# genlm/genlm-backend

Measured on AMD Instinct MI355X. Metric: particles/sec + logprob-kernel HBM GB/s (% of 8 TB/s), 1024 particles gpt2, higher is better.
Workload: dtype f32

## Files before the change

### genlm-backend_amd/_lib.py

```python
import ctypes as C
import os

_HERE = os.path.dirname(os.path.abspath(__file__))
LIB_PATH = os.path.join(_HERE, "libglb_hip.so")

ABI_VERSION = 9
GLB_OK, GLB_EINVAL, GLB_EUNSUPPORTED, GLB_EHIP, GLB_ENOSPC = 0, 1, 2, 3, 4
F32, BF16, F16 = 0, 1, 2
MASK_NONE, MASK_BITS, MASK_F32, MASK_PREPARED = 0, 1, 2, 3
RNG_NONE, RNG_PHILOX, RNG_NOISE = 0, 1, 2
STEP_HW_EXP = 1
GEMM_BIAS, GEMM_BIAS_GELU_TANH = 0, 1
GEMM_FORM_LARGE, GEMM_FORM_SMALL = 1, 2


class GlbError(RuntimeError):
    def __init__(self, code, msg):
        super().__init__(f"glb error {code}: {msg}")
        self.code = code


class StepArgs(C.Structure):
    _fields_ = [
        ("struct_size", C.c_uint32),
# ... 91 lines not shown
        ("workspace_bytes", C.c_size_t),
    ]


class KvPlanArgs(C.Structure):
    _fields_ = [
        ("struct_size", C.c_uint32),
        ("n", C.c_int64), ("n_rows", C.c_int64), ("cap", C.c_int64),
        ("group_of", C.c_void_p), ("rep", C.c_void_p), ("n_groups", C.c_void_p),
        ("old_row", C.c_void_p),
        ("old_row_by_context", C.c_int32),
        ("lengths", C.c_void_p),
        ("row_stamps", C.c_void_p),
        ("call_no", C.c_int64),
        ("row_tok", C.c_void_p), ("row_len", C.c_void_p),
        ("row_hash", C.c_void_p),
        ("group_hash", C.c_void_p),
        ("tokens", C.c_void_p),
        ("starts", C.c_void_p),
        ("out_group_row", C.c_void_p), ("out_logits_row", C.c_void_p), ("out_rows_a", C.c_void_p), ("out_ctx_a", C.c_void_p),
        ("out_pos_a", C.c_void_p), ("out_ctx_b", C.c_void_p), ("out_rows_b", C.c_void_p), ("out_copy_src", C.c_void_p),
        ("out_copy_len", C.c_void_p), ("out_ctx_of_row", C.c_void_p), ("out_pos_of_row", C.c_void_p),
        ("out_row_of_context", C.c_void_p), ("out_head", C.c_void_p),
        ("workspace", C.c_void_p),
        ("workspace_bytes", C.c_size_t),
    ]


class KvPlanChunkArgs(C.Structure):
    _fields_ = [
        ("struct_size", C.c_uint32),
        ("plan", KvPlanArgs),
        ("old_keep", C.c_void_p),
        ("out_n_new_a", C.c_void_p), ("out_n_new_of_row", C.c_void_p),
    ]


KV_CHUNK_MAX = 16


class MT19937(C.Structure):
    _fields_ = [("mt", C.c_uint32 * 624), ("idx", C.c_int32)]


MT_POLY_WORDS = 312


class MtRowsArgs(C.Structure):
    _fields_ = [
        ("struct_size", C.c_uint32),
        ("window", C.c_void_p), ("window_out", C.c_void_p), ("polys", C.c_void_p),
        ("n_small", C.c_int32), ("n_big", C.c_int32),
        ("vocab", C.c_int64), ("max_draw_rows", C.c_int64),
        ("n_draw", C.c_void_p),
        ("n_out_rows", C.c_int64),
        ("row_slot", C.c_void_p),
        ("out", C.c_void_p), ("out_ld", C.c_int64),
        ("workspace", C.c_void_p), ("workspace_bytes", C.c_size_t),
        ("reuse_windows", C.c_int32), ("rows_from", C.c_void_p), ("rows_from_ld", C.c_int64),
    ]


class GemmArgs(C.Structure):
    _fields_ = [
        ("struct_size", C.c_uint32),
        ("m", C.c_int64), ("n", C.c_int64), ("k", C.c_int64),
        ("a", C.c_void_p), ("lda", C.c_int64),
        ("w_split", C.c_void_p),
        ("bias", C.c_void_p),
        ("c", C.c_void_p), ("ldc", C.c_int64),
        ("epilogue", C.c_int32),
    ]


class PackedPlanArgs(C.Structure):
    _fields_ = [
        ("struct_size", C.c_uint32),
        ("n_tokens", C.c_int64), ("n_contexts", C.c_int64), ("n_sel", C.c_int64), ("n_groups", C.c_int64),
        ("n_pre", C.c_int64), ("n_tail_rows", C.c_int64), ("pos_cap", C.c_int64),
        ("tokens", C.c_void_p), ("starts", C.c_void_p), ("lengths", C.c_void_p), ("sel", C.c_void_p), ("grp", C.c_void_p),
        ("group_starts", C.c_void_p), ("group_lens", C.c_void_p), ("group_segments", C.c_void_p),
        ("group_ids", C.c_void_p), ("group_pos", C.c_void_p),
        ("segments", C.c_void_p), ("ids", C.c_void_p), ("pos", C.c_void_p), ("last", C.c_void_p), ("ends", C.c_void_p),
    ]


class LoraJob(C.Structure):
    _fields_ = [
        ("struct_size", C.c_uint32),
        ("w_dtype", C.c_int32), ("ab_dtype", C.c_int32), ("w_transposed", C.c_int32),
        ("n_out", C.c_int64), ("k_in", C.c_int64), ("r", C.c_int64),
        ("w", C.c_void_p), ("ldw", C.c_int64),
        ("a", C.c_void_p), ("lda", C.c_int64),
        ("b", C.c_void_p), ("ldb", C.c_int64),
        ("scale", C.c_float),
        ("out", C.c_void_p), ("ldo", C.c_int64),
    ]


class LoraRowsEntry(C.Structure):
    _fields_ = [
        ("struct_size", C.c_uint32),
        ("ab_dtype", C.c_int32),
        ("n_out", C.c_int64), ("k_in", C.c_int64), ("r", C.c_int64),
        ("a", C.c_void_p), ("lda", C.c_int64),
        ("b", C.c_void_p), ("ldb", C.c_int64),
        ("scale", C.c_float),
    ]


class LoraRowsArgs(C.Structure):
    _fields_ = [
        ("struct_size", C.c_uint32),
        ("dtype", C.c_int32),
        ("m", C.c_int64), ("n", C.c_int64), ("k", C.c_int64),
        ("x", C.c_void_p), ("ldx", C.c_int64),
        ("y", C.c_void_p), ("ldy", C.c_int64),
        ("row_slot", C.c_void_p),
        ("table", C.c_void_p),
        ("n_slots", C.c_int32), ("n_modules", C.c_int32), ("module", C.c_int32), ("r_max", C.c_int32),
        ("workspace", C.c_void_p), ("workspace_bytes", C.c_size_t),
    ]


class W4Args(C.Structure):
    _fields_ = [
        ("struct_size", C.c_uint32),
        ("dtype", C.c_int32), ("transposed", C.c_int32),
        ("n", C.c_int64), ("k", C.c_int64),
        ("w", C.c_void_p), ("ldw", C.c_int64),
        ("codebook", C.POINTER(C.c_float)),
        ("image", C.c_void_p), ("image_bytes", C.c_size_t),
    ]


class W4GemmArgs(C.Structure):
    _fields_ = [
        ("struct_size", C.c_uint32),
        ("dtype", C.c_int32),
        ("m", C.c_int64), ("n", C.c_int64), ("k", C.c_int64),
        ("x", C.c_void_p), ("ldx", C.c_int64),
        ("image", C.c_void_p),
        ("codebook", C.POINTER(C.c_float)),
        ("bias", C.c_void_p),
        ("y", C.c_void_p), ("ldy", C.c_int64),
        ("workspace", C.c_void_p), ("workspace_bytes", C.c_size_t),
    ]


DFA_COUNTERS = 4


class DfaArgs(C.Structure):
    _fields_ = [
        ("struct_size", C.c_uint32),
        ("n_states", C.c_int32), ("start", C.c_int32), ("eos_id", C.c_int32),
        ("delta", C.c_void_p), ("accepting", C.c_void_p), ("live", C.c_void_p),
        ("vocab", C.c_int64),
        ("tok_bytes", C.c_void_p), ("n_bytes", C.c_int64), ("tok_ptr", C.c_void_p), ("skip", C.c_void_p),
        ("n", C.c_int64),
        ("tokens", C.c_void_p), ("ld", C.c_int64), ("from_", C.c_void_p), ("to", C.c_void_p),
        ("state_in", C.c_void_p), ("state_out", C.c_void_p),
        ("bank", C.c_void_p), ("bank_ld", C.c_int64), ("capacity", C.c_int64),
        ("row_of_state", C.c_void_p), ("work", C.c_void_p), ("counters", C.c_void_p),
        ("max_work", C.c_int64),
        ("done", C.c_void_p), ("out_rows", C.c_void_p),
# ... 214 lines not shown
        ("seq_start", C.c_void_p), ("n_seq", C.c_int64),
        ("out_seq_logp", C.c_void_p), ("out_seq_logZ", C.c_void_p), ("out_seq_logp_masked", C.c_void_p),
    ]


class TopkArgs(C.Structure):
    _fields_ = [
        ("struct_size", C.c_uint32),
        ("logits", C.c_void_p), ("dtype", C.c_int32),
        ("n_rows", C.c_int64), ("vocab", C.c_int64), ("ld", C.c_int64),
        ("logit_scale", C.c_float), ("k", C.c_int32),
        ("mask_kind", C.c_int32), ("mask", C.c_void_p), ("mask_ld", C.c_int64), ("n_masks", C.c_int64),
        ("row_mask_id", C.c_void_p),
        ("out_token", C.c_void_p), ("out_logp", C.c_void_p), ("out_logp_masked", C.c_void_p),
        ("out_lse", C.c_void_p), ("out_logZ", C.c_void_p),
    ]


class ByteLmArgs(C.Structure):
    _fields_ = [
        ("struct_size", C.c_uint32), ("width", C.c_int32),
        ("n_groups", C.c_int64), ("n_nodes", C.c_int64), ("root", C.c_int32),
        ("child_ptr", C.c_void_p), ("child_idx", C.c_void_p), ("child_sym", C.c_void_p), ("leaf_token", C.c_void_p),
        ("node", C.c_void_p), ("alive", C.c_void_p), ("u", C.c_void_p), ("w", C.c_void_p),
        ("sel", C.c_void_p), ("mass", C.c_void_p), ("fresh", C.c_void_p),
        ("out_parent", C.c_void_p), ("out_token", C.c_void_p), ("out_node", C.c_void_p), ("out_alive", C.c_void_p),
        ("out_u", C.c_void_p), ("out_w", C.c_void_p), ("out_spawned", C.c_void_p), ("out_n_spawned", C.c_void_p),
        ("byte", C.c_void_p), ("out_next", C.c_void_p), ("out_logZ", C.c_void_p), ("logp", C.c_void_p),
    ]


class TruncateArgs(C.Structure):
    _fields_ = [
        ("struct_size", C.c_uint32),
        ("logits", C.c_void_p), ("dtype", C.c_int32),
        ("n_rows", C.c_int64), ("vocab", C.c_int64), ("ld", C.c_int64),
        ("logit_scale", C.c_float),
        ("mask_kind", C.c_int32), ("mask", C.c_void_p), ("mask_ld", C.c_int64), ("n_masks", C.c_int64),
        ("row_mask_id", C.c_void_p),
        ("top_k", C.c_int64), ("top_p", C.c_float), ("log_min_p", C.c_float),
        ("out_bits", C.c_void_p), ("out_ld", C.c_int64),
        ("out_threshold", C.c_void_p), ("out_kept", C.c_void_p), ("out_logmass", C.c_void_p),
    ]


_vp, _i32, _i64, _f32, _sz = C.c_void_p, C.c_int32, C.c_int64, C.c_float, C.c_size_t
SYMBOLS = {
    "glb_version": (C.c_char_p, []),
    "glb_abi_version": (C.c_int, []),
    "glb_last_error": (C.c_int, [C.c_char_p, _sz]),
    "glb_device_count": (C.c_int, []),
    "glb_step_workspace_bytes": (_sz, [_i64, _i64, _i64, _i64]),
    "glb_logprob_mask_sample": (C.c_int, [C.POINTER(StepArgs), _vp]),
    "glb_logprob_mask_sample_timed": (C.c_int, [C.POINTER(StepArgs), _vp, _vp, _vp]),
    "glb_workspace_init": (C.c_int, [_vp, _sz, _vp]),
    "glb_workspace_release": (C.c_int, [_vp]),
    "glb_workspace_check": (C.c_int, [_vp, _vp]),
    "glb_workspace_error_word": (_vp, [_vp]),
    "glb_set_spin_limit": (C.c_int, [C.c_uint64]),
    "glb_mask_prepared_bytes": (_sz, [_i64, _i64]),
    "glb_mask_prepare": (C.c_int, [_vp, _i64, _i64, _i64, _i32, _vp, _sz, _vp]),
    "glb_mask_prepare_rows": (C.c_int, [_vp, _i64, _i64, _i64, _i32, _vp, _i64, _vp, _sz, _vp]),
    "glb_log_softmax_workspace_bytes": (_sz, [_i64, _i64]),
    "glb_log_softmax_rows": (C.c_int, [_vp, _i32, _i64, _i64, _i64, _f32, _vp, _i32, _i64, _vp, _vp, _sz, _vp]),
    "glb_mask_f32_to_bits": (C.c_int, [_vp, _i64, _i64, _i64, _vp, _i64, _vp, _vp]),
    "glb_group_contexts_workspace": (_sz, [_i64]),
    "glb_group_contexts": (C.c_int, [_vp, _vp, _vp, _i64, _vp, _vp, _vp, _vp, _vp, _sz, _vp]),
    "glb_hash_contexts": (C.c_int, [_vp, _vp, _vp, _i64, _vp, _vp]),
    "glb_match_prefixes": (C.c_int, [_vp, _vp, _vp, _i64, _vp, _vp, _vp, _i64, _vp, _vp, _vp]),
    "glb_gather_padded": (C.c_int, [_vp, _vp, _vp, _vp, _i64, _vp, _i64, _i64, _i64, _vp, _vp, _vp, _vp, _vp]),
    "glb_gather_kv_padded": (C.c_int, [_vp, _vp, _i64, _vp, _i64, _i64, _i64, _i64, _i32, _vp, _vp]),
    "glb_particles_advance": (C.c_int, [_vp, _i64, _vp, _vp, _vp, _vp, _vp, _i64, _i32, _i32, _vp, _vp]),
    "glb_normalize_weights": (C.c_int, [_vp, _i64, _vp, _vp, _vp]),
    "glb_kv_append": (C.c_int, [_vp, _vp, _vp, _vp, _i64, _i64, _i64, _i64, _i64, _i64, _i32, _vp]),
    "glb_kv_gather_rows": (C.c_int, [_vp, _vp, _i64, _i64, _i64, _i64, _i64, _i64, _vp, _vp, _i32, _vp]),
    "glb_gather_rows_i32": (C.c_int, [_vp, _i64, _vp, _i64, _i64, _vp, _i64, _vp]),
    "glb_match_rows": (C.c_int, [_vp, _vp, _vp, _vp, _vp, _i64, _vp, _vp, _vp, _i64, _i64, _vp, _vp, _vp]),
    "glb_slab_attention": (C.c_int, [_vp, _i64, _i64, _vp, _i64, _i64, _vp, _i64, _i64, _vp, _vp, _vp, _i64, _i64, _i64, _i64, _i64,
                                     _f32, _i32, _vp, _vp]),
    "glb_short_attention": (C.c_int, [_vp, C.POINTER(C.c_int64), _vp, C.POINTER(C.c_int64), _vp, C.POINTER(C.c_int64), _vp, _i64, _i64,
                                      _i64, _i64, _i64, _i64, _i64, _i64, _f32, _i32, _vp, _vp]),
    "glb_short_attention_packed": (C.c_int, [_vp, _i64, _i64, _vp, _i64, _i64, _vp, _i64, _i64, _vp, _i64, _i64, _i64, _i64, _i64,
                                             _i64, _f32, _i32, _vp, _vp, _vp]),
    "glb_kv_plan_workspace": (_sz, [_i64, _i64]),
    "glb_kv_plan": (C.c_int, [C.POINTER(KvPlanArgs), _vp]),
    "glb_match_prefix_rows": (C.c_int, [_vp, _vp, _vp, _vp, _vp, _i64, _vp, _vp, _vp, _i64, _i64, _i32, _vp, _vp, _vp, _vp]),
    "glb_kv_plan_chunk": (C.c_int, [C.POINTER(KvPlanChunkArgs), _vp]),
    "glb_slab_attention_chunk": (C.c_int, [_vp, C.POINTER(C.c_int64), _vp, C.POINTER(C.c_int64), _vp, C.POINTER(C.c_int64), _vp, _vp,
                                           _vp, _vp, _vp, _i64, _i64, _i64, _i64, _i64, _i64, _i64, _f32, _i32, _vp, _vp]),
    "glb_trie_workspace": (_sz, [_i64, _i64]),
    "glb_trie_reduce": (C.c_int, [_vp, _i64, _i64, _i64, _i64, _i64, _vp, _vp, _vp, _vp, _vp, _i32, _i32, _vp, _i64, _vp, _sz,
                                  _vp]),
    "glb_trie_workspace_ex": (_sz, [_i64, _i64]),
    "glb_trie_masses": (C.c_int, [C.POINTER(TrieArgs), _vp]),
    "glb_trie_rows_workspace": (_sz, [_i64, C.POINTER(TriePlan)]),
    "glb_trie_rows": (C.c_int, [C.POINTER(TrieRowsArgs), C.POINTER(TriePlan), _vp]),
    "glb_resample_workspace": (_sz, [_i64]),
    "glb_resample_systematic": (C.c_int, [_vp, _i64, C.c_uint64, C.c_uint64, _vp, _vp, _vp, _sz, _vp]),
    "glb_mt19937_seed": (None, [C.POINTER(MT19937), C.c_uint64]),
    "glb_mt19937_exponential_f32": (C.c_int, [C.POINTER(MT19937), _vp, _i64]),
    "glb_mt19937_window": (C.c_int, [C.c_uint64, _vp]),
    "glb_mt19937_jump_polys": (C.c_int, [_i64, _i32, _i32, _vp]),
    "glb_mt19937_jump_host": (C.c_int, [_vp, _vp, _vp]),
    "glb_mt19937_rows_workspace": (_sz, [_i64, _i32]),
    "glb_mt19937_exponential_rows": (C.c_int, [C.POINTER(MtRowsArgs), _vp]),
    "glb_comm_unique_id": (C.c_int, [_vp]),
    "glb_comm_init": (C.c_int, [_vp, _i32, _i32, C.POINTER(C.c_void_p)]),
    "glb_allgather_f32": (C.c_int, [_vp, _vp, _i64, _vp, _vp]),
    "glb_comm_destroy": (C.c_int, [_vp]),
    "glb_gemm_split_bytes": (_sz, [_i64, _i64]),
    "glb_gemm_split_weights": (C.c_int, [_vp, _i64, _i64, _i64, _vp, _sz, _vp]),
    "glb_gemm_f32_split": (C.c_int, [C.POINTER(GemmArgs), _vp]),
    "glb_gemm_split_pick": (C.c_int, [_i64, _i64, _i64, C.c_int, C.POINTER(C.c_int)]),
    "glb_gemm_f32_split_form": (C.c_int, [C.POINTER(GemmArgs), C.c_int, _vp]),
    "glb_gemm_f32_split_residual": (C.c_int, [C.POINTER(GemmArgs), _vp, _i64, C.c_int, _vp]),
    "glb_packed_plan": (C.c_int, [C.POINTER(PackedPlanArgs), _vp]),
    "glb_gemm_split_blocks_per_cu": (C.c_int, [C.c_int, C.POINTER(C.c_int)]),
    "glb_gemm_split_form_blocks_per_cu": (C.c_int, [C.c_int, C.c_int, C.POINTER(C.c_int)]),
    "glb_lora_merge_workspace_bytes": (_sz, [_i32]),
    "glb_lora_merge": (C.c_int, [C.POINTER(LoraJob), _i32, _vp, _sz, _vp]),
    "glb_lora_rows_table_bytes": (_sz, [_i32, _i32]),
    "glb_lora_rows_table_upload": (C.c_int, [C.POINTER(LoraRowsEntry), _i32, _i32, _vp, _sz, _vp]),
    "glb_lora_rows_workspace_bytes": (_sz, [_i64, _i32]),
    "glb_lora_rows": (C.c_int, [C.POINTER(LoraRowsArgs), _vp]),
    "glb_w4_bytes": (_sz, [_i64, _i64]),
    "glb_w4_quantize": (C.c_int, [C.POINTER(W4Args), _vp]),
    "glb_w4_dequantize": (C.c_int, [C.POINTER(W4Args), _vp]),
    "glb_w4_gemm_max_rows": (C.c_int, []),
    "glb_w4_gemm_workspace_bytes": (_sz, [_i64, _i64, _i64]),
    "glb_w4_gemm": (C.c_int, [C.POINTER(W4GemmArgs), _vp]),
    "glb_dfa_bank_init": (C.c_int, [C.POINTER(DfaArgs), _vp]),
    "glb_dfa_advance": (C.c_int, [C.POINTER(DfaArgs), _vp]),
    "glb_dfa_claim_rows": (C.c_int, [C.POINTER(DfaArgs), _vp]),
    "glb_dfa_fill_masks": (C.c_int, [C.POINTER(DfaArgs), _vp]),
    "glb_dfa_mask_ids": (C.c_int, [C.POINTER(DfaArgs), _vp]),
    "glb_dfa_bank_rows": (_i64, [_sz, _i64, _i64]),
    "glb_dfa_weight_bank_init": (C.c_int, [C.POINTER(DfaWeightArgs), _vp]),
    "glb_dfa_fill_weights": (C.c_int, [C.POINTER(DfaWeightArgs), _vp]),
    "glb_dfa_weight_bank_rows": (_i64, [_sz, _i64, _i64]),
    "glb_dfa_evict_bank_init": (C.c_int, [C.POINTER(DfaEvictArgs), _vp]),
    "glb_dfa_evict_serve": (C.c_int, [C.POINTER(DfaEvictArgs), _vp]),
    "glb_dfa_backward": (C.c_int, [C.POINTER(DfaPushArgs), _vp]),
    "glb_dfa_push_weights": (C.c_int, [C.POINTER(DfaPushArgs), _vp]),
    "glb_dfa_refine": (C.c_int, [C.POINTER(DfaMinArgs), _vp]),
    "glb_dfa_quotient": (C.c_int, [C.POINTER(DfaMinArgs), _vp]),
    "glb_fsa_product_round": (C.c_int, [C.POINTER(FsaProductArgs), _vp]),
    "glb_fsa_live": (C.c_int, [C.POINTER(FsaProductArgs), _vp]),
    "glb_nfa_closure": (C.c_int, [C.POINTER(NfaArgs), _vp]),
    "glb_nfa_subset_round": (C.c_int, [C.POINTER(NfaArgs), _vp]),
    "glb_lazy_init": (C.c_int, [C.POINTER(LazyArgs), _vp]),
    "glb_lazy_advance": (C.c_int, [C.POINTER(LazyArgs), _vp]),
    "glb_lazy_serve": (C.c_int, [C.POINTER(LazyArgs), _vp]),
    "glb_pda_init": (C.c_int, [C.POINTER(PdaArgs), _vp]),
    "glb_pda_advance": (C.c_int, [C.POINTER(PdaArgs), _vp]),
    "glb_pda_serve": (C.c_int, [C.POINTER(PdaArgs), _vp]),
    "glb_conj_init": (C.c_int, [C.POINTER(ConjArgs), _vp]),
    "glb_conj_unpack": (C.c_int, [C.POINTER(ConjArgs), _vp]),
    "glb_conj_number": (C.c_int, [C.POINTER(ConjArgs), _vp]),
    "glb_conj_serve": (C.c_int, [C.POINTER(ConjArgs), _vp]),
    "glb_importance_workspace_bytes": (_sz, [_i64, _i64, _i64]),
    "glb_importance_step": (C.c_int, [C.POINTER(ImportanceArgs), _vp]),
    "glb_score_rows": (C.c_int, [C.POINTER(ScoreArgs), _vp]),
    "glb_score_seq_sums": (C.c_int, [_vp, _i64, _vp, _i64, _vp, _vp]),
    "glb_topk_rows": (C.c_int, [C.POINTER(TopkArgs), _vp]),
    "glb_truncate_rows": (C.c_int, [C.POINTER(TruncateArgs), _vp]),
    "glb_beam_select": (C.c_int, [_vp, _vp, _vp, _vp, _i64, _i32, _i32, _vp, _vp, _vp, _vp]),
    "glb_bytelm_children": (C.c_int, [C.POINTER(ByteLmArgs), _vp]),
    "glb_bytelm_extend": (C.c_int, [C.POINTER(ByteLmArgs), _vp]),
    "glb_bytelm_next": (C.c_int, [C.POINTER(ByteLmArgs), _vp]),
    "glb_philox4x32_10": (None, [C.POINTER(C.c_uint32), C.POINTER(C.c_uint32), C.POINTER(C.c_uint32)]),
}

_lib = None


def load():
    global _lib
    if _lib is not None:
        return _lib
    if not os.path.exists(LIB_PATH):
        raise ImportError(
            f"{LIB_PATH} not found: build it with `make -C genlm-backend_amd/csrc -j8` "
            "(or `python -c 'import __graft_entry__ as g; g.build()'`). There is no CPU fallback."
        )
    import torch

    lib = C.CDLL(LIB_PATH)
    for name, (res, args) in SYMBOLS.items():
        fn = getattr(lib, name)
        fn.restype = res
        fn.argtypes = args
    if lib.glb_abi_version() != ABI_VERSION:
        raise ImportError(f"libglb_hip.so ABI {lib.glb_abi_version()} != {ABI_VERSION}")
    _lib = lib
    return lib


def last_error():
    buf = C.create_string_buffer(512)
# ... 8 lines not shown
```

### genlm-backend_amd/csrc/glb_kv.hip

```cpp
#include <hip/hip_runtime.h>

#include <climits>

#include "../../include/glb.h"
#include "glb_common.hpp"

namespace {

__device__ inline uint64_t ctx_hash_step(uint64_t h, uint32_t v) {
  h ^= v;
  h *= 0x100000001b3ull;
  return h ^ (h >> 29);
}

__global__ __launch_bounds__(64) void match_rows_kernel(const int32_t *tok, const int64_t *st, const int32_t *len,
                                                        const int32_t *rep, const int32_t *n_groups, const int32_t *row_tok,
                                                        const int32_t *row_len, const uint64_t *row_hash, int32_t R,
                                                        int32_t cap, int32_t *out_old, uint64_t *out_hash) {
  const int u = blockIdx.x, lane = threadIdx.x;
  if (u >= *n_groups) return;
  const int i = rep[u];
  const int32_t L = len[i];
  const int32_t *t = tok + st[i];
  uint64_t h = 0xcbf29ce484222325ull, h_par = h;
// ... 717 lines not shown
    const int qc = live ? qi : nq - 1;
    const int g = qc / a.Lq, t = qc - g * a.Lq, h = hk * G + g;
    float qf[EPV];
    unpack16<DT>(q_raw, qf);
    if (q0 + PP < nq) q_raw = *reinterpret_cast<const u32x4 *>(q_addr(qi + PP));
    const uint32_t vis = vis_t[t];
    float sc[KMAX];
    float m = -__builtin_huge_valf();
#pragma unroll
    for (int p = 0; p < KMAX; ++p) {
      sc[p] = -__builtin_huge_valf();
      if (p < a.Lk) {
        float s = 0.0f;
        if constexpr (KREG) {
#pragma unroll
          for (int k = 0; k < EPV; ++k) s = __builtin_fmaf(qf[k], kr[p][k], s);
        } else {
          const float *kp = Ks + p * DH + i * EPV;
#pragma unroll
          for (int k = 0; k < EPV; ++k) s = __builtin_fmaf(qf[k], kp[k], s);
        }
        s = slot_sum<LP>(s) * a.scale;
        sc[p] = ((vis >> p) & 1u) ? s : -__builtin_huge_valf();
        m = fmaxf(m, sc[p]);
      }
    }
    float l = 0.0f, acc[EPV];
#pragma unroll
    for (int k = 0; k < EPV; ++k) acc[k] = 0.0f;
#pragma unroll
    for (int p = 0; p < KMAX; ++p) {
      if (p < a.Lk) {
        const float w = ((vis >> p) & 1u) ? __expf(sc[p] - m) : 0.0f;
        const float *vp = Vs + p * DH + i * EPV;
        l += w;
#pragma unroll
        for (int k = 0; k < EPV; ++k) acc[k] = __builtin_fmaf(w, vp[k], acc[k]);
      }
    }
    if (live) {
      const float inv = l > 0.0f ? 1.0f / l : 0.0f;
#pragma unroll
      for (int k = 0; k < EPV; ++k) acc[k] *= inv;
      *reinterpret_cast<u32x4 *>(a.out + ((((int64_t)u * a.Lq + t) * a.H + h) * DH + i * EPV) * ES) = pack16v<DT>(acc);
    }
  }
}

template <int DT, int DH>
hipError_t launch_short_rows(const ShortArgs &a, hipStream_t s) {
  const dim3 grid((unsigned)((int64_t)a.U * a.Hkv)), block(64);
  const size_t lds = (size_t)2 * a.Lk * DH * sizeof(float) + (size_t)a.Lq * sizeof(uint32_t);
  if (a.Lk <= 16) hipLaunchKernelGGL((short_attention_rows_kernel<DT, DH, 16>), grid, block, lds, s, a);
  else hipLaunchKernelGGL((short_attention_rows_kernel<DT, DH, 32>), grid, block, lds, s, a);
  return hipGetLastError();
}

template <int DT>
hipError_t launch_short_attention(const ShortArgs &a, int head_dim, hipStream_t s) {
  if (a.Lk <= 32 && a.Lq <= 2048 && (int64_t)a.U * a.Hkv <= 0x7fffffffll) {
    if (head_dim == 64) return launch_short_rows<DT, 64>(a, s);
    if (head_dim == 128) return launch_short_rows<DT, 128>(a, s);
    if (head_dim == 32) return launch_short_rows<DT, 32>(a, s);
    if (head_dim == 16) return launch_short_rows<DT, 16>(a, s);
    return hipErrorInvalidValue;
  }
  const dim3 grid((unsigned)((int64_t)a.U * a.H * a.Lq)), block(64);
  if (head_dim == 64) hipLaunchKernelGGL((short_attention_kernel<DT, 64>), grid, block, 0, s, a);
  else if (head_dim == 128) hipLaunchKernelGGL((short_attention_kernel<DT, 128>), grid, block, 0, s, a);
  else if (head_dim == 32) hipLaunchKernelGGL((short_attention_kernel<DT, 32>), grid, block, 0, s, a);
  else if (head_dim == 16) hipLaunchKernelGGL((short_attention_kernel<DT, 16>), grid, block, 0, s, a);
  else return hipErrorInvalidValue;
  return hipGetLastError();
}

struct PackedArgs {
  const char *q, *k, *v;
  char *out;
  const int32_t *plan;
  uint32_t *err;
  int64_t q_sr, q_sh, k_sr, k_sh, v_sr, v_sh;
  int32_t S, M, H, Hkv, max_keys;
  float scale;
};

template <int DT, int DH, int KMAX>
__global__ __launch_bounds__(64) void short_attention_packed_kernel(const PackedArgs a) {
  constexpr int ES = DT == GLB_F32 ? 4 : 2, EPV = 16 / ES, LP = DH / EPV, PP = 64 / LP;
  static_assert(LP >= 1 && LP <= 64 && PP * LP == 64, "head_dim / vector width must divide the wave");
  constexpr bool KREG = KMAX * EPV <= 128;
  extern __shared__ float kv_lds[];
  const int lane = threadIdx.x, j = lane / LP, i = lane - j * LP;
  const int G = a.H / a.Hkv;
  const int hk = blockIdx.x % a.Hkv, s = blockIdx.x / a.Hkv;
  if (s >= a.S) return;
  const int32_t *seg = a.plan + (int64_t)s * 4;
  const int64_t pre_start = seg[0], pre_len = seg[1], tail_start = seg[2], tail_len = seg[3];
  const int64_t n_keys = pre_len + tail_len;
  if (pre_len < 0 || tail_len < 1 || n_keys > a.max_keys || n_keys > KMAX || pre_start < 0 || pre_start + pre_len > a.M ||
      tail_start < 0 || tail_start + tail_len > a.M) {
    if (lane == 0 && hk == 0) atomicAdd(a.err, 1u);
    return;
  }
  const int Lk = (int)n_keys, Lq = (int)tail_len, pre = (int)pre_len;
  auto key_row = [&](int p) -> int64_t { return p < pre ? pre_start + p : tail_start + (p - pre); };
  float *Ks = kv_lds, *Vs = KREG ? kv_lds : kv_lds + Lk * DH;
  const char *kb = a.k + (int64_t)hk * a.k_sh * ES;
  const char *vb = a.v + (int64_t)hk * a.v_sh * ES;
  const int nq = G * Lq;
  auto q_addr = [&](int qi) {
    const int qc = qi < nq ? qi : nq - 1;
    const int g = qc / Lq, t = qc - g * Lq;
    return a.q + ((tail_start + t) * a.q_sr + (int64_t)(hk * G + g) * a.q_sh + i * EPV) * ES;
  };
  u32x4 q_raw = *reinterpret_cast<const u32x4 *>(q_addr(j));
  float kr[KREG ? KMAX : 1][EPV];
  if constexpr (KREG) {
    u32x4 raw[KMAX];
#pragma unroll
    for (int p = 0; p < KMAX; ++p)
      raw[p] = *reinterpret_cast<const u32x4 *>(kb + (key_row(p < Lk ? p : 0) * a.k_sr + i * EPV) * ES);
#pragma unroll
    for (int p = 0; p < KMAX; ++p) unpack16<DT>(raw[p], kr[p]);
  }
  for (int x = lane; x < Lk * LP; x += 64) {
    const int p = x / LP, c = x - p * LP;
    const int64_t row = key_row(p);
    float vf[EPV];
    unpack16<DT>(*reinterpret_cast<const u32x4 *>(vb + (row * a.v_sr + c * EPV) * ES), vf);
#pragma unroll
    for (int k = 0; k < EPV; ++k) Vs[p * DH + c * EPV + k] = vf[k];
    if constexpr (!KREG) {
      float kf[EPV];
      unpack16<DT>(*reinterpret_cast<const u32x4 *>(kb + (row * a.k_sr + c * EPV) * ES), kf);
#pragma unroll
      for (int k = 0; k < EPV; ++k) Ks[p * DH + c * EPV + k] = kf[k];
    }
  }
  const uint32_t all_keys = Lk >= 32 ? 0xffffffffu : ((1u << Lk) - 1u);
  uint32_t *vis_t = reinterpret_cast<uint32_t *>(kv_lds + (KREG ? 1 : 2) * Lk * DH);
  for (int t = lane; t < Lq; t += 64) {
    const int last = t + pre;
    const uint32_t vis = last >= 31 ? 0xffffffffu : ((2u << last) - 1u);
    vis_t[t] = vis & all_keys;
  }
  __syncthreads();
  for (int q0 = 0; q0 < nq; q0 += PP) {
    const int qi = q0 + j;
    const bool live = qi < nq;
    const int qc = live ? qi : nq - 1;
    const int g = qc / Lq, t = qc - g * Lq, h = hk * G + g;
    float qf[EPV];
    unpack16<DT>(q_raw, qf);
    if (q0 + PP < nq) q_raw = *reinterpret_cast<const u32x4 *>(q_addr(qi + PP));
    const uint32_t vis = vis_t[t];
    float sc[KMAX];
    float m = -__builtin_huge_valf();
#pragma unroll
    for (int p = 0; p < KMAX; ++p) {
      sc[p] = -__builtin_huge_valf();
      if (p < Lk) {
        float sv = 0.0f;
        if constexpr (KREG) {
#pragma unroll
          for (int k = 0; k < EPV; ++k) sv = __builtin_fmaf(qf[k], kr[p][k], sv);
        } else {
          const float *kp = Ks + p * DH + i * EPV;
#pragma unroll
          for (int k = 0; k < EPV; ++k) sv = __builtin_fmaf(qf[k], kp[k], sv);
        }
        sv = slot_sum<LP>(sv) * a.scale;
        sc[p] = ((vis >> p) & 1u) ? sv : -__builtin_huge_valf();
        m = fmaxf(m, sc[p]);
      }
    }
    float l = 0.0f, acc[EPV];
#pragma unroll
    for (int k = 0; k < EPV; ++k) acc[k] = 0.0f;
#pragma unroll
    for (int p = 0; p < KMAX; ++p) {
      if (p < Lk) {
// ... 319 lines not shown
  p.lengths = a->lengths;
  p.stamps = a->row_stamps;
  p.call_no = a->call_no;
  p.grp_row = a->out_group_row;
  p.inv = a->out_logits_row;
  p.rows_a = a->out_rows_a;
  p.reps_a = a->out_ctx_a;
  p.pos_a = a->out_pos_a;
  p.reps_b = a->out_ctx_b;
  p.rows_b = a->out_rows_b;
  p.copy_src = a->out_copy_src;
  p.copy_len = a->out_copy_len;
  p.ctx_of_row = a->out_ctx_of_row;
  p.pos_full = a->out_pos_of_row;
  p.row_of_new = a->out_row_of_context;
  p.head = a->out_head;
  p.row_tok = a->row_tok;
  p.row_len = a->row_len;
  p.row_hash = a->row_hash;
  p.grp_hash = a->group_hash;
  p.tok = a->tokens;
  p.st = a->starts;
  p.old_keep = old_keep;
  p.n_new_a = n_new_a;
  p.n_new_row = n_new_row;
  int32_t *ws = (int32_t *)a->workspace;
  p.keeper = ws;
  p.free_by_rank = ws + a->n_rows;
  p.flags = ws + 2 * a->n_rows;
  p.lds_rows = a->row_stamps && a->n_rows <= 15360 ? (int32_t)a->n_rows : 0;
  hipLaunchKernelGGL(kv_plan_kernel, dim3(1), dim3(kT), (size_t)p.lds_rows * sizeof(int), (hipStream_t)stream, p);
  const hipError_t e = hipGetLastError();
  if (e != hipSuccess) return glb::api_hip_fail(e, "kv_plan launch");
  return GLB_OK;
}

int glb_short_attention(const void *q, const int64_t q_strides[3], const void *k, const int64_t k_strides[3], const void *v,
                        const int64_t v_strides[3], const uint8_t *mask, int64_t mask_stride_row, int64_t mask_stride_query,
                        int64_t n_rows, int64_t heads, int64_t kv_heads, int64_t q_len, int64_t k_len, int64_t head_dim,
                        float scale, int32_t dtype, void *out, void *stream) {
  if (!q || !k || !v || !out || !q_strides || !k_strides || !v_strides) return glb::api_fail(GLB_EINVAL, "glb_short_attention: null pointer");
  if (dtype < GLB_F32 || dtype > GLB_F16) return glb::api_fail(GLB_EINVAL, "bad dtype %d", dtype);
  if (n_rows <= 0 || heads <= 0 || kv_heads <= 0 || q_len <= 0 || k_len <= 0 || heads % kv_heads || k_len < q_len ||
      n_rows * heads * q_len > 0x7fffffffll || k_len > 0x7fffffffll)
    return glb::api_fail(GLB_EINVAL, "glb_short_attention: bad sizes");
  if (head_dim != 16 && head_dim != 32 && head_dim != 64 && head_dim != 128)
    return glb::api_fail(GLB_EUNSUPPORTED, "glb_short_attention: head_dim %lld (16, 32, 64 and 128 are built)", (long long)head_dim);
  const int es = dtype == GLB_F32 ? 4 : 2;
  bool aligned = (((uintptr_t)q | (uintptr_t)k | (uintptr_t)v | (uintptr_t)out) % 16) == 0;
  for (int d = 0; d < 3; ++d) aligned = aligned && (q_strides[d] * es) % 16 == 0 && (k_strides[d] * es) % 16 == 0 && (v_strides[d] * es) % 16 == 0;
  if (!aligned) return glb::api_fail(GLB_EINVAL, "glb_short_attention: pointers and strides must be 16-byte aligned");
  ShortArgs a{};
  a.q = (const char *)q;
  a.k = (const char *)k;
  a.v = (const char *)v;
  a.mask = mask;
  a.out = (char *)out;
  a.q_sr = q_strides[0], a.q_sh = q_strides[1], a.q_sp = q_strides[2];
  a.k_sr = k_strides[0], a.k_sh = k_strides[1], a.k_sp = k_strides[2];
  a.v_sr = v_strides[0], a.v_sh = v_strides[1], a.v_sp = v_strides[2];
  a.m_sr = mask_stride_row;
  a.m_sq = mask_stride_query;
  a.U = (int32_t)n_rows;
  a.H = (int32_t)heads;
  a.Hkv = (int32_t)kv_heads;
  a.Lq = (int32_t)q_len;
  a.Lk = (int32_t)k_len;
  a.scale = scale;
  hipError_t e;
  switch (dtype) {
    case GLB_F32: e = launch_short_attention<GLB_F32>(a, (int)head_dim, (hipStream_t)stream); break;
    case GLB_BF16: e = launch_short_attention<GLB_BF16>(a, (int)head_dim, (hipStream_t)stream); break;
    default: e = launch_short_attention<GLB_F16>(a, (int)head_dim, (hipStream_t)stream); break;
  }
  if (e != hipSuccess) return glb::api_hip_fail(e, "short_attention launch");
  return GLB_OK;
}

int glb_short_attention_packed(const void *q, int64_t q_stride_row, int64_t q_stride_head, const void *k, int64_t k_stride_row,
                               int64_t k_stride_head, const void *v, int64_t v_stride_row, int64_t v_stride_head,
                               const int32_t *plan, int64_t n_segments, int64_t n_rows, int64_t heads, int64_t kv_heads,
                               int64_t max_keys, int64_t head_dim, float scale, int32_t dtype, void *out, uint32_t *err_word,
                               void *stream) {
  if (!q || !k || !v || !out || !plan || !err_word) return glb::api_fail(GLB_EINVAL, "glb_short_attention_packed: null pointer");
  if (dtype < GLB_F32 || dtype > GLB_F16) return glb::api_fail(GLB_EINVAL, "bad dtype %d", dtype);
  if (n_segments <= 0 || n_rows <= 0 || heads <= 0 || kv_heads <= 0 || heads % kv_heads || heads > 0x7fffffffll ||
      n_rows > 0x7fffffffll || n_segments > 0x7fffffffll || n_segments * kv_heads > 0x7fffffffll)
    return glb::api_fail(GLB_EINVAL, "glb_short_attention_packed: bad sizes");
  if (max_keys < 1 || max_keys > 32)
    return glb::api_fail(GLB_EINVAL, "glb_short_attention_packed: %lld keys per context (1 .. 32 are served)", (long long)max_keys);
  if (head_dim != 16 && head_dim != 32 && head_dim != 64 && head_dim != 128)
    return glb::api_fail(GLB_EUNSUPPORTED, "glb_short_attention_packed: head_dim %lld (16, 32, 64 and 128 are built)", (long long)head_dim);
  const int es = dtype == GLB_F32 ? 4 : 2;
  bool aligned = (((uintptr_t)q | (uintptr_t)k | (uintptr_t)v | (uintptr_t)out | (uintptr_t)plan) % 16) == 0 && ((uintptr_t)err_word % 4) == 0;
  for (int64_t st : {q_stride_row, q_stride_head, k_stride_row, k_stride_head, v_stride_row, v_stride_head})
    aligned = aligned && st >= 0 && (st * es) % 16 == 0;
  if (!aligned) return glb::api_fail(GLB_EINVAL, "glb_short_attention_packed: pointers and strides must be 16-byte aligned");
  PackedArgs a{};
  a.q = (const char *)q;
  a.k = (const char *)k;
  a.v = (const char *)v;
  a.out = (char *)out;
  a.plan = plan;
  a.err = err_word;
  a.q_sr = q_stride_row, a.q_sh = q_stride_head;
  a.k_sr = k_stride_row, a.k_sh = k_stride_head;
  a.v_sr = v_stride_row, a.v_sh = v_stride_head;
  a.S = (int32_t)n_segments;
  a.M = (int32_t)n_rows;
  a.H = (int32_t)heads;
  a.Hkv = (int32_t)kv_heads;
  a.max_keys = (int32_t)max_keys;
  a.scale = scale;
  hipError_t e;
  switch (dtype) {
    case GLB_F32: e = launch_short_packed<GLB_F32>(a, (int)head_dim, (hipStream_t)stream); break;
    case GLB_BF16: e = launch_short_packed<GLB_BF16>(a, (int)head_dim, (hipStream_t)stream); break;
    default: e = launch_short_packed<GLB_F16>(a, (int)head_dim, (hipStream_t)stream); break;
  }
  if (e != hipSuccess) return glb::api_hip_fail(e, "short_attention_packed launch");
  return GLB_OK;
}

}
```

### genlm-backend_amd/csrc/glb_packed_plan.hip

```cpp
#include <hip/hip_runtime.h>

#include <cstdint>

#include "../../include/glb.h"
#include "glb_common.hpp"

namespace {

constexpr int SCAN_THREADS = 1024, ROW_THREADS = 256;

__device__ __forceinline__ int32_t wrap_add(int32_t a, int32_t b) { return (int32_t)((uint32_t)a + (uint32_t)b); }
__device__ __forceinline__ int32_t wrap_sub(int32_t a, int32_t b) { return (int32_t)((uint32_t)a - (uint32_t)b); }

__device__ __forceinline__ int64_t ctx_index(int32_t s, int64_t n) {
  int64_t i = s < 0 ? (int64_t)s + n : (int64_t)s;
  return i < 0 ? 0 : (i >= n ? n - 1 : i);
}

__global__ __launch_bounds__(SCAN_THREADS) void packed_plan_scan_kernel(glb_packed_plan_args a) {
  __shared__ int32_t wave_sum[SCAN_THREADS / 64];
  __shared__ int32_t carry_s;
  const int tid = threadIdx.x, lane = tid & 63, wave = tid >> 6;
  const int64_t G = a.n_groups, U = a.n_sel;
  for (int64_t i = tid; i < G * 4; i += SCAN_THREADS) a.segments[i] = a.group_segments[i];
  if (tid == 0) carry_s = 0;
  __syncthreads();
  for (int64_t base = 0; base < U; base += SCAN_THREADS) {
    const int64_t u = base + tid;
    int32_t pre_len = 0, pre_start = 0, tail = 0;
    if (u < U) {
      int64_t g = a.grp[u];
      g = g < 0 ? 0 : (g > G - 1 ? G - 1 : g);
      pre_len = a.group_lens[g];
      pre_start = a.group_starts[g];
      tail = wrap_sub(a.lengths[ctx_index(a.sel[u], a.n_contexts)], pre_len);
    }
    int32_t x = tail;
#pragma unroll
    for (int d = 1; d < 64; d <<= 1) {
      const int32_t y = __shfl_up(x, d, 64);
      if (lane >= d) x = wrap_add(x, y);
    }
    if (lane == 63) wave_sum[wave] = x;
    __syncthreads();
    int32_t before = carry_s;
    for (int w = 0; w < wave; ++w) before = wrap_add(before, wave_sum[w]);
    const int32_t end = wrap_add(before, x);
    if (u < U) {
      const int32_t tail_start = wrap_sub(wrap_add((int32_t)a.n_pre, end), tail);
      a.ends[u] = end;
      int32_t *seg = a.segments + (G + u) * 4;
      seg[0] = pre_start;
      seg[1] = pre_len;
      seg[2] = tail_start;
      seg[3] = tail;
      const int64_t last = (int64_t)wrap_sub(wrap_add(tail_start, tail), 1), m = a.n_pre + a.n_tail_rows;
      a.last[u] = last < 0 ? 0 : (last > m - 1 ? m - 1 : last);
    }
    __syncthreads();
    if (tid == SCAN_THREADS - 1) carry_s = end;
    __syncthreads();
  }
}

__global__ __launch_bounds__(ROW_THREADS) void packed_plan_rows_kernel(glb_packed_plan_args a) {
  const int64_t row = (int64_t)blockIdx.x * ROW_THREADS + threadIdx.x;
  if (row >= a.n_pre + a.n_tail_rows) return;
  if (row < a.n_pre) {
    a.ids[row] = a.group_ids[row];
    a.pos[row] = a.group_pos[row];
    return;
  }
  const int64_t U = a.n_sel;
  const int32_t r = (int32_t)(row - a.n_pre);
  int64_t lo = 0, hi = U;
  while (lo < hi) {
    const int64_t mid = lo + ((hi - lo) >> 1);
    if (a.ends[mid] > r) hi = mid; else lo = mid + 1;
  }
  const int64_t u = lo > U - 1 ? U - 1 : lo;
  const int32_t *seg = a.segments + (a.n_groups + u) * 4;
  const int32_t pos_t = wrap_add(seg[1], wrap_sub(r, wrap_sub(a.ends[u], seg[3])));
  int64_t at = a.starts[ctx_index(a.sel[u], a.n_contexts)] + (int64_t)pos_t;
  at = at < 0 ? 0 : (at > a.n_tokens - 1 ? a.n_tokens - 1 : at);
  a.ids[row] = (int64_t)a.tokens[at];
  const int64_t p = pos_t;
  a.pos[row] = p < 0 ? 0 : (p > a.pos_cap - 1 ? a.pos_cap - 1 : p);
}

}

extern "C" int glb_packed_plan(const glb_packed_plan_args *args, void *stream) {
  if (!args) return glb::api_fail(GLB_EINVAL, "glb_packed_plan: null argument block");
  if (args->struct_size != sizeof(glb_packed_plan_args))
    return glb::api_fail(GLB_EINVAL, "glb_packed_plan_args.struct_size %u != %zu (ABI mismatch)", args->struct_size,
                         sizeof(glb_packed_plan_args));
  const glb_packed_plan_args &a = *args;
  if (a.n_groups < 1 || a.n_sel < 1 || a.n_pre < 1 || a.n_tail_rows < a.n_sel || a.n_contexts < 1 || a.n_tokens < 1 ||
      a.pos_cap < 1 || a.n_sel > INT32_MAX || a.n_pre + a.n_tail_rows > INT32_MAX)
    return glb::api_fail(GLB_EINVAL, "glb_packed_plan: bad sizes (G %lld, U %lld, prompt rows %lld, tail rows %lld, contexts %lld, "
                         "tokens %lld, position cap %lld)", (long long)a.n_groups, (long long)a.n_sel, (long long)a.n_pre,
                         (long long)a.n_tail_rows, (long long)a.n_contexts, (long long)a.n_tokens, (long long)a.pos_cap);
  if (!a.tokens || !a.starts || !a.lengths || !a.sel || !a.grp || !a.group_starts || !a.group_lens || !a.group_segments ||
      !a.group_ids || !a.group_pos)
    return glb::api_fail(GLB_EINVAL, "glb_packed_plan: null input");
  if (!a.segments || !a.ids || !a.pos || !a.last || !a.ends) return glb::api_fail(GLB_EINVAL, "glb_packed_plan: null output");
  hipStream_t s = (hipStream_t)stream;
  hipLaunchKernelGGL(packed_plan_scan_kernel, dim3(1), dim3(SCAN_THREADS), 0, s, a);
  hipError_t e = hipGetLastError();
  if (e != hipSuccess) return glb::api_hip_fail(e, "glb_packed_plan scan launch");
  hipLaunchKernelGGL(packed_plan_rows_kernel, dim3(blocks_for(a.n_pre + a.n_tail_rows, ROW_THREADS)), dim3(ROW_THREADS), 0, s, a);
  e = hipGetLastError();
  if (e != hipSuccess) return glb::api_hip_fail(e, "glb_packed_plan rows launch");
  return GLB_OK;
}
```

### genlm-backend_amd/engine.py

```python
import ctypes as C

import numpy as np
import torch

from . import _lib
from ._lib import GLB_EHIP, GlbError
from ._lib import (F32, BF16, F16, MASK_NONE, MASK_BITS, MASK_F32, MASK_PREPARED, RNG_NONE, RNG_PHILOX, RNG_NOISE,
                   STEP_HW_EXP, KvPlanArgs, KvPlanChunkArgs, MtRowsArgs, StepArgs, TrieArgs, TriePlan, TrieRowsArgs, MT19937, MT_POLY_WORDS, check)

_DT = {torch.float32: F32, torch.bfloat16: BF16, torch.float16: F16}


def _ptr(t):
    return None if t is None else C.c_void_p(t.data_ptr())


class LoraRowsTable:

    def __init__(self, dev, n_slots, n_modules, r_max, keep):
        self.dev, self.n_slots, self.n_modules, self.r_max, self.keep = dev, n_slots, n_modules, r_max, keep


class HostRng:

# ... 799 lines not shown
        if w.device != self.device:
            raise ValueError(f"tensor on {w.device}, engine on {self.device}")
        out =torch.empty(nbytes, dtype=torch.uint8, device=self.device)
        check(self.lib.glb_gemm_split_weights(_ptr(w), k, n, w.stride(0), _ptr(out), nbytes, self._stream()))
        return out

    def gemm_split(self, x, w_split, n, bias=None, gelu=False, out=None, form=None, residual=None):
        k = x.shape[-1]
        x2 = x.reshape(-1, k)
        m = x2.shape[0]
        if m == 0 or x2.stride(1) != 1:
            return None
        if bias is not None:
            if bias.device != self.device:
                raise ValueError(f"bias on {bias.device}, engine on {self.device}")
            if bias.dim() != 1 or bias.numel() != n:
                raise ValueError(f"bias of shape {tuple(bias.shape)}, expected ({n},)")
            if bias.dtype != torch.float32 or bias.stride(0) != 1:
                return None
        if out is None:
            out = torch.empty((m, n), dtype=torch.float32, device=self.device)
        else:
            if out.device != self.device:
                raise ValueError(f"out on {out.device}, engine on {self.device}")
            if out.dtype != torch.float32 or tuple(out.shape) != (m, n):
                raise ValueError(f"out is {out.dtype} {tuple(out.shape)}, expected torch.float32 {(m, n)}")
            if out.stride(1) != 1 or (m > 1 and out.stride(0) < n):
                raise ValueError(f"out has strides {out.stride()}: rows of unit inner stride, at least {n} apart, are needed")
        a = _lib.GemmArgs()
        a.struct_size = C.sizeof(_lib.GemmArgs)
        a.m, a.n, a.k = m, n, k
        a.a, a.lda = x2.data_ptr(), x2.stride(0)
        a.w_split = w_split.data_ptr()
        a.bias = bias.data_ptr() if bias is not None else None
        a.c, a.ldc = out.data_ptr(), max(out.stride(0), n)
        a.epilogue = _lib.GEMM_BIAS_GELU_TANH if gelu else _lib.GEMM_BIAS
        if residual is not None:
            if gelu:
                raise ValueError("gemm_split: the residual epilogue does not follow the GELU")
            if residual.device != self.device:
                raise ValueError(f"residual on {residual.device}, engine on {self.device}")
            r2 = residual.view(-1, n) if residual.dim() != 2 else residual
            if residual.dtype != torch.float32 or tuple(r2.shape) != (m, n) or r2.stride(1) != 1 or (m > 1 and r2.stride(0) < n):
                raise ValueError(f"residual is {residual.dtype} {tuple(residual.shape)} with strides {residual.stride()}: "
                                 f"torch.float32 {(m, n)} rows of unit inner stride are needed")
            rc = self.lib.glb_gemm_f32_split_residual(C.byref(a), r2.data_ptr(), max(r2.stride(0), n), int(form or 0),
                                                      self._stream())
        elif form is None:
            rc = self.lib.glb_gemm_f32_split(C.byref(a), self._stream())
        else:
            rc = self.lib.glb_gemm_f32_split_form(C.byref(a), int(form), self._stream())
        if rc == _lib.GLB_EUNSUPPORTED:
            return None
        check(rc)
        return out.view(*x.shape[:-1], n)

    def packed_plan(self, batch, sel, n_sel, grp, groups, n_tail_rows, pos_cap):
        tokens, starts, lengths = batch
        G, n_pre = len(groups.lens), groups.n_rows
        ins = (tokens, starts, lengths, sel, grp, groups.starts_d, groups.lens_d, groups.segments, groups.ids, groups.pos)
        self._check_dev(*ins)
        want = (torch.int32, torch.int64, torch.int32, torch.int32, torch.int32, torch.int32, torch.int32, torch.int32,
                torch.int64, torch.int64)
        if any(t.dtype != d for t, d in zip(ins, want)):
            raise ValueError(f"packed_plan: dtypes {[t.dtype for t in ins]}, expected {list(want)}")
        if sel.numel() < n_sel or grp.numel() < n_sel or starts.numel() != lengths.numel() or groups.ids.numel() != n_pre:
            raise ValueError("packed_plan: sel / grp shorter than n_sel, or starts / lengths / the prompts' rows disagree")
        M = n_pre + int(n_tail_rows)
        seg = torch.empty((G + n_sel, 4), dtype=torch.int32, device=self.device)
        ids = torch.empty(M, dtype=torch.int64, device=self.device)
        pos = torch.empty(M, dtype=torch.int64, device=self.device)
        last = torch.empty(n_sel, dtype=torch.int64, device=self.device)
        ends = self._i32(n_sel)
        a = _lib.PackedPlanArgs()
        a.struct_size = C.sizeof(_lib.PackedPlanArgs)
        a.n_tokens, a.n_contexts, a.n_sel, a.n_groups = tokens.numel(), lengths.numel(), n_sel, G
        a.n_pre, a.n_tail_rows, a.pos_cap = n_pre, int(n_tail_rows), int(pos_cap)
        (a.tokens, a.starts, a.lengths, a.sel, a.grp, a.group_starts, a.group_lens, a.group_segments, a.group_ids,
         a.group_pos) = (t.data_ptr() for t in ins)
        a.segments, a.ids, a.pos, a.last, a.ends = (t.data_ptr() for t in (seg, ids, pos, last, ends))
        check(self.lib.glb_packed_plan(C.byref(a), self._stream()))
        return seg, ids, pos, last

    def lora_merge(self, jobs):
        n = len(jobs)
        if n == 0:
            return
        table = (_lib.LoraJob * n)()
        for q, j in zip(table, jobs):
            w, a, b, out = j["w"], j["a"], j["b"], j["out"]
            for t in (w, a, b, out):
                if t.device != self.device:
                    raise ValueError(f"tensor on {t.device}, engine on {self.device}")
                if t.dim() != 2 or t.stride(1) != 1:
                    raise ValueError("lora_merge: every matrix must be 2-D with unit inner stride")
                if t.dtype not in _DT:
                    raise ValueError(f"lora_merge: unsupported dtype {t.dtype}")
            if a.dtype != b.dtype or out.dtype != w.dtype or out.shape != w.shape:
                raise ValueError("lora_merge: a / b must share a dtype, out must match w's dtype and shape")
            tr = bool(j.get("transposed", False))
            q.struct_size = C.sizeof(_lib.LoraJob)
            q.w_dtype, q.ab_dtype, q.w_transposed = _DT[w.dtype], _DT[a.dtype], int(tr)
            q.k_in, q.n_out = (w.shape[0], w.shape[1]) if tr else (w.shape[1], w.shape[0])
            q.r = a.shape[0]
            if tuple(a.shape) != (q.r, q.k_in) or tuple(b.shape) != (q.n_out, q.r):
                raise ValueError(f"lora_merge: a {tuple(a.shape)} / b {tuple(b.shape)} do not fit w {tuple(w.shape)}")
            q.w, q.ldw = w.data_ptr(), w.stride(0)
            q.a, q.lda = a.data_ptr(), a.stride(0)
            q.b, q.ldb = b.data_ptr(), b.stride(0)
            q.scale = float(j["scale"])
            q.out, q.ldo = out.data_ptr(), out.stride(0)
        nbytes = self.lib.glb_lora_merge_workspace_bytes(n)
        ws = torch.empty(nbytes, dtype=torch.uint8, device=self.device)
        check(self.lib.glb_lora_merge(table, n, _ptr(ws), nbytes, self._stream()))

    def lora_rows_table(self, slots):
        n_slots = len(slots)
        n_modules = len(slots[0]) if n_slots else 0
        nbytes = self.lib.glb_lora_rows_table_bytes(n_slots, n_modules)
        if nbytes == 0:
            raise ValueError(f"lora_rows_table: {n_slots} slots x {n_modules} modules is not served")
        host = (_lib.LoraRowsEntry * (n_slots * n_modules))()
        keep, r_max = [], 0
        for si, mods in enumerate(slots):
            if len(mods) != n_modules:
                raise ValueError("lora_rows_table: every slot lists every module")
            for mi, j in enumerate(mods):
                q = host[si * n_modules + mi]
                q.struct_size = C.sizeof(_lib.LoraRowsEntry)
                if j is None:
                    continue
                a, b = j["a"], j["b"]
                for t in (a, b):
                    if t.device != self.device:
                        raise ValueError(f"tensor on {t.device}, engine on {self.device}")
                    if t.dim() != 2 or t.stride(1) != 1 or t.dtype not in _DT:
                        raise ValueError("lora_rows_table: a / b must be 2-D float32 / bfloat16 / float16 with unit inner stride")
                if a.dtype != b.dtype or a.shape[0] != b.shape[1]:
                    raise ValueError("lora_rows_table: a / b must share a dtype and the rank")
                q.ab_dtype = _DT[a.dtype]
                q.n_out, q.k_in, q.r = b.shape[0], a.shape[1], a.shape[0]
                q.a, q.lda = a.data_ptr(), a.stride(0)
                q.b, q.ldb = b.data_ptr(), b.stride(0)
                q.scale = float(j["scale"])
                keep += [a, b]
                r_max = max(r_max, int(a.shape[0]))
        dev = torch.empty(nbytes, dtype=torch.uint8, device=self.device)
        check(self.lib.glb_lora_rows_table_upload(host, n_slots, n_modules, _ptr(dev), nbytes, self._stream()))
        return LoraRowsTable(dev, n_slots, n_modules, max(r_max, 1), keep)

    @staticmethod
    def _rows_2d(t, what):
        if t.dim() < 1 or t.stride(-1) != 1:
            raise ValueError(f"lora_rows: {what} must have unit inner stride")
        rows, pitch = 1, None
        for d in range(t.dim() - 2, -1, -1):
            if t.shape[d] == 1:
                continue
            if pitch is None:
                pitch = t.stride(d)
            elif t.stride(d) != pitch * rows:
                raise ValueError(f"lora_rows: {what} is not a matrix of rows with one pitch")
            rows *= t.shape[d]
        return rows, (t.shape[-1] if pitch is None else pitch)

    def lora_rows(self, x, y, row_slot, table, module_index):
# ... 114 lines not shown
        if name not in HipEngine.DFA_CALLS:
            raise ValueError(name)
        check(getattr(self.lib, name)(C.byref(args), self._stream()))

    FSA_CALLS = frozenset(name for name, (_, argtypes) in _lib.SYMBOLS.items()
                          if name.startswith("glb_fsa_") and argtypes and issubclass(argtypes[0], C._Pointer))

    def fsa_call(self, name, args):
        if name not in HipEngine.FSA_CALLS:
            raise ValueError(name)
        check(getattr(self.lib, name)(C.byref(args), self._stream()))

    NFA_CALLS = frozenset(name for name, (_, argtypes) in _lib.SYMBOLS.items()
                          if name.startswith("glb_nfa_") and argtypes and issubclass(argtypes[0], C._Pointer))

    def nfa_call(self, name, args):
        if name not in HipEngine.NFA_CALLS:
            raise ValueError(name)
        check(getattr(self.lib, name)(C.byref(args), self._stream()))

    LAZY_CALLS = frozenset(name for name, (_, argtypes) in _lib.SYMBOLS.items()
                           if name.startswith("glb_lazy_") and argtypes and issubclass(argtypes[0], C._Pointer))

    def lazy_call(self, name, args):
        if name not in HipEngine.LAZY_CALLS:
            raise ValueError(name)
        check(getattr(self.lib, name)(C.byref(args), self._stream()))

    PDA_CALLS = frozenset(name for name, (_, argtypes) in _lib.SYMBOLS.items()
                          if name.startswith("glb_pda_") and argtypes and issubclass(argtypes[0], C._Pointer))

    def pda_call(self, name, args):
        if name not in HipEngine.PDA_CALLS:
            raise ValueError(name)
        check(getattr(self.lib, name)(C.byref(args), self._stream()))

    CONJ_CALLS = frozenset(name for name, (_, argtypes) in _lib.SYMBOLS.items()
                           if name.startswith("glb_conj_") and argtypes and issubclass(argtypes[0], C._Pointer))

    def conj_call(self, name, args):
        if name not in HipEngine.CONJ_CALLS:
            raise ValueError(name)
        check(getattr(self.lib, name)(C.byref(args), self._stream()))

    def kv_append(self, slab, new_rows, pos, rows=None):
        R, H, cap, Dh = slab.shape
        n = new_rows.shape[0]
        assert new_rows.shape == (n, H, 1, Dh) and new_rows.stride(3) == 1 and slab.is_contiguous()
        assert rows is not None or n == R
        check(self.lib.glb_kv_append(_ptr(slab), _ptr(new_rows), _ptr(pos), _ptr(rows), n, H, cap, Dh, new_rows.stride(0),
                                     new_rows.stride(1), slab.element_size(), self._stream()))

    def slab_attention(self, query, k_new, v_new, k_slab, v_slab, pos, scale):
        R, H, _, Dh = query.shape
        Hkv, cap = k_slab.shape[1], k_slab.shape[2]
        assert query.stride(3) == 1 and k_new.stride(3) == 1 and v_new.stride(3) == 1 and k_slab.is_contiguous() and v_slab.is_contiguous()
        assert k_new.dtype == v_new.dtype == query.dtype == k_slab.dtype
        out = torch.empty((R, 1, H, Dh), dtype=query.dtype, device=self.device)
        check(self.lib.glb_slab_attention(_ptr(query), query.stride(0), query.stride(1), _ptr(k_new), k_new.stride(0),
                                          k_new.stride(1), _ptr(v_new), v_new.stride(0), v_new.stride(1), _ptr(k_slab),
                                          _ptr(v_slab), _ptr(pos), R, H, Hkv,
                                          cap, Dh, float(scale), _DT[query.dtype], _ptr(out), self._stream()))
        return out

    @staticmethod
    def slab_attention_supports(dtype, head_dim):
        return dtype in _DT and head_dim in (16, 32, 64, 128)

    def short_attention(self, query, key, value, mask, scale):
        U, H, Lq, Dh = query.shape
        Hkv, Lk = key.shape[1], key.shape[2]
        assert query.stride(3) == 1 and key.stride(3) == 1 and value.stride(3) == 1 and key.dtype == value.dtype == query.dtype
        out = torch.empty((U, Lq, H, Dh), dtype=query.dtype, device=self.device)
        i64x3 = C.c_int64 * 3
        m_ptr, m_sr, m_sq = None, 0, 0
        if mask is not None:
            assert mask.dtype == torch.bool and mask.dim() == 4 and mask.shape[-1] == Lk and mask.stride(3) == 1 and mask.shape[1] == 1
            m_ptr, m_sr, m_sq = _ptr(mask), (mask.stride(0) if mask.shape[0] > 1 else 0), (mask.stride(2) if mask.shape[2] > 1 else 0)
        check(self.lib.glb_short_attention(_ptr(query), i64x3(*query.stride()[:3]), _ptr(key), i64x3(*key.stride()[:3]), _ptr(value),
                                           i64x3(*value.stride()[:3]), m_ptr, m_sr, m_sq, U, H, Hkv, Lq, Lk, Dh, float(scale),
                                           _DT[query.dtype], _ptr(out), self._stream()))
        return out

    def short_attention_packed(self, query, key, value, plan, max_keys, scale, err=None, out=None):
        M, H, Dh = query.shape
        Hkv = key.shape[1]
        assert key.shape == value.shape == (M, Hkv, Dh) and key.dtype == value.dtype == query.dtype
        assert query.stride(2) == 1 and key.stride(2) == 1 and value.stride(2) == 1
        assert plan.dtype == torch.int32 and plan.dim() == 2 and plan.shape[1] == 4 and plan.is_contiguous()
        self._check_dev(plan)
        err = self.error_word() if err is None else err
        assert err.dtype == torch.int32 and err.device == self.device
        if out is None:
            out = torch.empty((M, H, Dh), dtype=query.dtype, device=self.device)
        assert out.shape == (M, H, Dh) and out.dtype == query.dtype and out.device == self.device and out.is_contiguous()
        check(self.lib.glb_short_attention_packed(_ptr(query), query.stride(0), query.stride(1), _ptr(key), key.stride(0),
                                                  key.stride(1), _ptr(value), value.stride(0), value.stride(1), _ptr(plan),
                                                  plan.shape[0], M, H, Hkv, int(max_keys), Dh, float(scale),
                                                  _DT[query.dtype], _ptr(out), _ptr(err), self._stream()))
        return out

    def kv_gather_rows(self, srcs, dsts, src_row_of, len_of, srcs_stable=True):
        s0, d0 = srcs[0], dsts[0]
        assert all(t.is_contiguous() for t in srcs) and all(t.is_contiguous() for t in dsts)
        sp = self._ptr_table(srcs) if srcs_stable else torch.tensor([t.data_ptr() for t in srcs], dtype=torch.int64, device=self.device)
        dp = self._ptr_table(dsts)
        check(self.lib.glb_kv_gather_rows(_ptr(sp), _ptr(dp), len(srcs), d0.shape[0], d0.shape[1], d0.shape[3],
                                          s0.shape[2], d0.shape[2], _ptr(src_row_of), _ptr(len_of), d0.element_size(),
                                          self._stream()))

    def _ptr_table(self, tensors):
        import weakref

        key = tuple(t.data_ptr() for t in tensors)
        ent = self._ptr_tables.get(key)
        if ent is not None and all(r() is t for r, t in zip(ent[1], tensors)):
            return ent[0]
        dead = [k for k, (_, refs) in self._ptr_tables.items() if any(r() is None for r in refs)]
        for k in dead:
            del self._ptr_tables[k]
        if len(self._ptr_tables) >= 64:
            self._ptr_tables.pop(next(iter(self._ptr_tables)))
        table = torch.tensor(key, dtype=torch.int64, device=self.device)
        self._ptr_tables[key] = (table, [weakref.ref(t) for t in tensors])
        return table

    def gather_rows_i32(self, src, row_of, out=None):
        n, width = row_of.numel(), src.shape[1]
        if out is None:
            out = torch.empty((n, width), dtype=torch.int32, device=self.device)
        check(self.lib.glb_gather_rows_i32(_ptr(src), src.stride(0), _ptr(row_of), n, width, _ptr(out), out.stride(0),
                                           self._stream()))
        return out

    def match_rows(self, tokens, starts, lengths, rep, n_groups, row_tok, row_len, row_hash):
        n = lengths.numel()
        R, cap = row_tok.shape
        self._check_dev(tokens, starts, lengths, rep, n_groups, row_tok, row_len, row_hash)
        old = self._i32(n)
        gh = torch.empty(n, dtype=torch.int64, device=self.device)
        check(self.lib.glb_match_rows(_ptr(tokens), _ptr(starts), _ptr(lengths), _ptr(rep), _ptr(n_groups), n, _ptr(row_tok),
                                      _ptr(row_len), _ptr(row_hash), R, cap, _ptr(old), _ptr(gh), self._stream()))
        return old, gh

    def kv_plan(self, group_of, rep, n_groups, old_row, lengths, n_rows, cap, by_context=False, stamps=None, call_no=0,
                table=None, old_keep=None):
        n = group_of.numel()
        self._check_dev(group_of, rep, n_groups, old_row, lengths, stamps, old_keep)
        chunk = old_keep is not None
        buf = torch.empty(9 * n + 5 * n_rows + 10 if chunk else 8 * n + 4 * n_rows + 8, dtype=torch.int32, device=self.device)
        names_n = ("group_row", "logits_row", "rows_a", "ctx_a", "pos_a", "ctx_b", "rows_b", "row_of_context")
        names_r = ("copy_src", "copy_len", "ctx_of_row", "pos_of_row")
        out, o = {}, 0
        if chunk:
            out["n_new_a"], out["n_new_of_row"], o = buf[:n], buf[n:n + n_rows], n + n_rows
        for k in names_n:
            out[k] = buf[o:o + n]
            o += n
        for k in names_r:
            out[k] = buf[o:o + n_rows]
            o += n_rows
        out["head"] = buf[o:o + (10 if chunk else 8)]
        need = self.lib.glb_kv_plan_workspace(n, n_rows)
        if self._ws is None or self._ws.numel() < need:
            self._ws = torch.empty(max(need, 1 << 16), dtype=torch.uint8, device=self.device)
        if chunk:
            c = KvPlanChunkArgs()
            c.struct_size = C.sizeof(KvPlanChunkArgs)
            c.old_keep, c.out_n_new_a, c.out_n_new_of_row = old_keep.data_ptr(), out["n_new_a"].data_ptr(), out["n_new_of_row"].data_ptr()
            a = c.plan
        else:
            a = KvPlanArgs()
        a.struct_size = C.sizeof(KvPlanArgs)
        a.n, a.n_rows, a.cap = n, n_rows, cap
        a.group_of, a.rep, a.n_groups = group_of.data_ptr(), rep.data_ptr(), n_groups.data_ptr()
        a.old_row, a.old_row_by_context = old_row.data_ptr(), 1 if by_context else 0
        a.lengths = lengths.data_ptr()
        a.row_stamps = None if stamps is None else stamps.data_ptr()
# ... 184 lines not shown
```

### genlm-backend_amd/kv.py

```python
import gc
import itertools
from collections import OrderedDict

import numpy as np
import torch
from transformers.cache_utils import Cache, CacheLayerMixin, DynamicCache


_ATTN_NAME = "glb"
SHORT_ATTENTION_MAX = 4096


def _glb_attention_forward(module, query, key, value, attention_mask, dropout=0.0, scaling=None, **kwargs):
    from transformers.integrations.sdpa_attention import sdpa_attention_forward

    layer = getattr(key, "_glb_layer", None)
    if layer is not None and layer._new_k is not None and getattr(layer.owner, "n_new", None) is not None:
        if key is not layer.keys or value is not layer.values:
            raise RuntimeError("glb_slab_attention_chunk: the attention module changed the key / value tensors the KV slab "
                               "handed out: the new tokens were never appended")
        k_new, v_new, layer._new_k, layer._new_v = layer._new_k, layer._new_v, None, None
        o = layer.owner
        scale = scaling if scaling is not None else query.shape[-1] ** -0.5
        return o.engine.slab_attention_chunk(query, k_new, v_new, layer.keys, layer.values, o.pos, o.n_new, scale, rows=o.rows), None
    if layer is not None and layer._new_k is not None:
        if key is not layer.keys or value is not layer.values or query.shape[2] != 1:
            raise RuntimeError("glb_slab_attention: the attention module changed the key / value tensors the KV slab handed "
                               "out (or feeds more than one token): the new token was never appended - run this model with "
                               "SlabForward(fused_attention=False)")
        k_new, v_new, layer._new_k, layer._new_v = layer._new_k, layer._new_v, None, None
        o = layer.owner
        scale = scaling if scaling is not None else query.shape[-1] ** -0.5
        return o.engine.slab_attention(query, k_new, v_new, layer.keys, layer.values, o.pos, scale), None
    packed = getattr(key, "_glb_packed", None)
    if packed is not None:
        if query.shape[0] != 1 or key.shape[2] != query.shape[2] or query.shape[2] != packed.n_rows or value.shape != key.shape:
            raise RuntimeError("glb_short_attention_packed: the attention module changed the shape of the packed batch")
        scale = scaling if scaling is not None else query.shape[-1] ** -0.5
        out = packed.engine.short_attention_packed(query[0].transpose(0, 1), key[0].transpose(0, 1), value[0].transpose(0, 1),
                                                   packed.segments, packed.max_keys, scale)
        packed.served += 1
        return out.unsqueeze(0), None
    eng = getattr(getattr(module, "config", None), "_glb_engine", None)
    Lq, Lk = query.shape[2], key.shape[2]
    wants_grad = torch.is_grad_enabled() and (query.requires_grad or key.requires_grad or value.requires_grad)
    if (eng is not None and query.is_cuda and not dropout and not wants_grad and not getattr(module, "training", False)
            and Lq * Lk <= SHORT_ATTENTION_MAX and Lk >= Lq
            and eng.slab_attention_supports(query.dtype, query.shape[-1]) and key.dtype == query.dtype == value.dtype
            and query.stride(3) == 1 and key.stride(3) == 1 and value.stride(3) == 1
            and kwargs.get("is_causal", True) is not False and not kwargs.get("softcap") and not kwargs.get("sliding_window")
            and getattr(module, "is_causal", True)
            and (attention_mask is None or (attention_mask.dtype == torch.bool and attention_mask.dim() == 4
                                            and attention_mask.shape[1] == 1 and attention_mask.shape[-1] == Lk
                                            and attention_mask.stride(3) == 1))
            and all((st * query.element_size()) % 16 == 0 for t in (query, key, value) for st in t.stride()[:3])
            and all(t.data_ptr() % 16 == 0 for t in (query, key, value))):
        scale = scaling if scaling is not None else query.shape[-1] ** -0.5
        return eng.short_attention(query, key, value, attention_mask, scale), None
    return sdpa_attention_forward(module, query, key, value, attention_mask, dropout=dropout, scaling=scaling, **kwargs)


def _register_attention():
    from transformers.masking_utils import ALL_MASK_ATTENTION_FUNCTIONS
    from transformers.modeling_utils import ALL_ATTENTION_FUNCTIONS

    if _ATTN_NAME not in ALL_ATTENTION_FUNCTIONS:
        ALL_ATTENTION_FUNCTIONS.register(_ATTN_NAME, _glb_attention_forward)
        ALL_MASK_ATTENTION_FUNCTIONS.register(_ATTN_NAME, ALL_MASK_ATTENTION_FUNCTIONS["sdpa"])


def use_glb_attention(shadow, engine):
    cfg = getattr(shadow, "config", None)
    if cfg is not None and getattr(cfg, "_attn_implementation", None) == _ATTN_NAME:
        return getattr(cfg, "_glb_engine", None) is engine
    if (cfg is None or not hasattr(engine, "short_attention") or getattr(cfg, "_attn_implementation", None) != "sdpa"
            or getattr(cfg, "attn_logit_softcapping", None) or getattr(cfg, "sliding_window", None)
            or getattr(cfg, "scale_attn_by_inverse_layer_idx", False)):
        return False
    _register_attention()
    cfg._attn_implementation = _ATTN_NAME
    cfg._glb_engine = engine
    return True


class _SlabLayer(CacheLayerMixin):

    is_compileable = False
    is_sliding = False

    def __init__(self, owner, idx):
        super().__init__()
        self.owner, self.idx = owner, idx
        self._new_k = self._new_v = None

    def lazy_initialization(self, key_states, value_states):
        o = self.owner
        shape_k = (o.n, key_states.shape[1], o.cap, key_states.shape[-1])
        shape_v = (o.n, value_states.shape[1], o.cap, value_states.shape[-1])
        self.keys = torch.zeros(shape_k, dtype=key_states.dtype, device=key_states.device)
        self.values = torch.zeros(shape_v, dtype=value_states.dtype, device=value_states.device)
        self.is_initialized = True

    def update(self, key_states, value_states, *args, **kwargs):
        if not self.is_initialized:
            self.lazy_initialization(key_states, value_states)
        o = self.owner
        if key_states.shape[0] != o.n or key_states.shape[-2] != 1:
            raise ValueError("SlabKV takes one new token for every particle per forward")
        if o.fused_attention:
            self._new_k, self._new_v = key_states, value_states
            self.keys._glb_layer = self
            return self.keys, self.values
        o.engine.kv_append(self.keys, key_states, o.pos)
        o.engine.kv_append(self.values, value_states, o.pos)
        return self.keys, self.values

    def get_mask_sizes(self, query_length):
        return self.owner.cap, 0

    def get_seq_length(self):
        return self.owner.cap - 1

    def get_max_length(self):
# ... 391 lines not shown

    def __init__(self, out, last):
        self.out, self.hidden, self.last = out, out.last_hidden_state, last

    def last_rows(self):
        return self.hidden[torch.arange(self.last.numel(), device=self.last.device), self.last.long()]

    def kv_layers(self):
        return [(ly.keys.contiguous(), ly.values.contiguous()) for ly in self.out.past_key_values.layers]


def encode_ragged(llm, batch, sel, n_sel, l_max, pad_id=0, base=None, prefixes=None, keep_kv=False):
    table, pref = prefixes or (None, None)
    eng = llm.engine
    ids, am, pos, last = eng.gather_padded(*batch, sel, n_sel, base, pad_id, 0 if table is None else table.p_max, l_max)
    cache = None if table is None else table.cache_for(eng, pref)
    return RaggedEncoding(llm._body(input_ids=ids, attention_mask=am, position_ids=pos, past_key_values=cache,
                                    use_cache=keep_kv or cache is not None), last)


PACKED_MAX_KEYS = 32


class PromptGroups:

    def __init__(self, prompts, device):
        if not prompts or any(len(p) < 1 for p in prompts):
            raise ValueError("a prompt group needs at least one token")
        self.lens = [len(p) for p in prompts]
        self.n_rows, self.p_max = sum(self.lens), max(self.lens)
        starts = np.concatenate([[0], np.cumsum(self.lens[:-1])]).astype(np.int32)
        lens = np.asarray(self.lens, np.int32)
        self.ids = torch.tensor([t for p in prompts for t in p], dtype=torch.int64, device=device)
        self.pos = torch.tensor([j for p in prompts for j in range(len(p))], dtype=torch.int64, device=device)
        self.starts_d, self.lens_d = torch.from_numpy(starts).to(device), torch.from_numpy(lens).to(device)
        zero = np.zeros_like(lens)
        self.segments = torch.from_numpy(np.stack([zero, zero, starts, lens], 1)).to(device)


def packed_plan(group_lens, grp, lens):
    group_lens, grp, lens = np.asarray(group_lens, np.int64), np.asarray(grp, np.int64), np.asarray(lens, np.int64)
    g_start = np.concatenate([[0], np.cumsum(group_lens[:-1])])
    n_pre = int(group_lens.sum())
    tail = lens - group_lens[grp]
    if (tail < 1).any():
        raise ValueError("every context needs a tail of at least one token behind its prompt")
    t_start = n_pre + np.concatenate([[0], np.cumsum(tail[:-1])])
    zero = np.zeros_like(group_lens)
    seg = np.concatenate([np.stack([zero, zero, g_start, group_lens], 1),
                          np.stack([g_start[grp], group_lens[grp], t_start, tail], 1)]).astype(np.int32)
    ctx = np.concatenate([np.repeat(-1 - np.arange(len(group_lens)), group_lens), np.repeat(np.arange(len(lens)), tail)])
    off = np.concatenate([np.arange(p) for p in group_lens] + [group_lens[grp[u]] + np.arange(tail[u]) for u in range(len(lens))])
    return seg, off.astype(np.int64), np.stack([ctx, off], 1).astype(np.int64), (t_start + tail - 1).astype(np.int64)


class _PackedLayer(CacheLayerMixin):

    is_compileable = False
    is_sliding = False

    def __init__(self, owner):
        super().__init__()
        self.owner = owner

    def lazy_initialization(self, key_states, value_states):
        self.is_initialized = True

    def update(self, key_states, value_states, *args, **kwargs):
        key_states._glb_packed = self.owner
        return key_states, value_states

    def get_mask_sizes(self, query_length):
        return query_length, 0

    def get_seq_length(self):
        return 0

    def get_max_length(self):
        return -1


class PackedKV(Cache):

    def __init__(self, engine, segments, n_rows, max_keys, n_layers):
        self.engine, self.segments, self.n_rows, self.max_keys = engine, segments, int(n_rows), int(max_keys)
        self.served = 0
        layer = _PackedLayer(self)
        super().__init__(layers=[layer] * n_layers)


class PackedEncoding:

    def __init__(self, out, last, n_rows):
        self.out, self.hidden, self.last, self.n_rows = out, out.last_hidden_state[0], last, n_rows

    def last_rows(self):
        return self.hidden[self.last]


def packed_supported(llm):
    body, eng = llm._body, llm.engine
    cfg = getattr(body, "config", None)
    if cfg is None or getattr(cfg, "_attn_implementation", None) != _ATTN_NAME or getattr(cfg, "_glb_engine", None) is not eng:
        return False
    heads = getattr(cfg, "num_attention_heads", None)
    head_dim = getattr(cfg, "head_dim", None) or (cfg.hidden_size // heads if heads else None)
    return bool(head_dim in (16, 32, 64, 128) and getattr(cfg, "num_hidden_layers", 0) > 0)


def _packed_plan_arrays(llm, batch, sel, n_sel, grp, groups, n_tail_rows, native_plan=True):
    eng, dev = llm.engine, llm.device
    tokens, starts, lengths = batch
    G, n_pre = len(groups.lens), groups.n_rows
    M = n_pre + int(n_tail_rows)
    max_pos = getattr(llm._body.config, "max_position_embeddings", None) or (1 << 30)
    pos_cap = min(PACKED_MAX_KEYS, max_pos)
    native = getattr(eng, "packed_plan", None) if native_plan else None
    if native is not None:
        return native(batch, sel, n_sel, grp, groups, n_tail_rows, pos_cap) + (M,)
    sel_l, grp_l = sel[:n_sel].long(), grp[:n_sel].long().clamp(0, G - 1)
    pre_len, pre_start = groups.lens_d[grp_l], groups.starts_d[grp_l]
    tail = lengths[sel_l] - pre_len
    ends = torch.cumsum(tail, 0, dtype=torch.int32)
    tail_start = n_pre + ends - tail
    segments = torch.cat([groups.segments, torch.stack([pre_start, pre_len, tail_start, tail], 1)]).contiguous()
    r = torch.arange(int(n_tail_rows), dtype=torch.int32, device=dev)
    u = torch.searchsorted(ends, r, right=True).clamp_(max=n_sel - 1)
    pos_t = (pre_len[u] + (r - (ends - tail)[u])).long()
    at = (starts[sel_l[u]] + pos_t).clamp_(0, tokens.numel() - 1)
    ids = torch.cat([groups.ids, tokens[at].long()])
    pos = torch.cat([groups.pos, pos_t.clamp_(0, pos_cap - 1)])
    return segments, ids, pos, (tail_start + tail - 1).long().clamp_(0, M - 1), M


def encode_packed(llm, batch, sel, n_sel, grp, groups, n_tail_rows, max_keys=PACKED_MAX_KEYS, native_plan=True):
    eng = llm.engine
    if not 1 <= max_keys <= PACKED_MAX_KEYS:
        raise ValueError(f"encode_packed serves contexts of up to {PACKED_MAX_KEYS} tokens")
    if n_sel < 1 or n_tail_rows < n_sel:
        raise ValueError("encode_packed: every context feeds at least one tail row")
    if not packed_supported(llm):
        raise RuntimeError("encode_packed: this model's attention is not served by glb_short_attention")
    segments, ids, pos, last, M = _packed_plan_arrays(llm, batch, sel, n_sel, grp, groups, n_tail_rows, native_plan)
    ids, pos = ids.view(1, M), pos.view(1, M)
    pkv = PackedKV(eng, segments, M, max_keys, llm._body.config.num_hidden_layers)
    out = llm._body(input_ids=ids, position_ids=pos, attention_mask=None, past_key_values=pkv, use_cache=True)
    if pkv.served != len(pkv.layers):
        raise RuntimeError(f"glb_short_attention_packed served {pkv.served} of {len(pkv.layers)} layers: an attention module "
                           "bypassed the attention interface and attended across the packed contexts")
    return PackedEncoding(out, last, M)


class PrefixLRU:

    def __init__(self, budget_bytes, on_remove=None):
        self.budget = int(budget_bytes)
        self.used = 0
        self._od = OrderedDict()
        self.evictions = 0
        self.on_remove = on_remove

    def put(self, node, kv):
        self.drop(node)
        size = kv.nbytes()
        node.past_key_values = kv
        self._od[id(node)] = (node, size)
        self.used += size
        while self.used > self.budget and len(self._od) > 1:
            _, (old, sz) = self._od.popitem(last=False)
            old.past_key_values = None
            self.used -= sz
            self.evictions += 1
            if self.on_remove is not None:
                self.on_remove(old)

    def touch(self, node):
        key = id(node)
        if key in self._od:
            self._od.move_to_end(key)

    def drop(self, node):
        ent = self._od.pop(id(node), None)
        if ent is not None:
            self.used -= ent[1]
            ent[0].past_key_values = None
            if self.on_remove is not None:
                self.on_remove(ent[0])

    def clear(self):
        nodes = [node for node, _ in self._od.values()]
        for node in nodes:
            node.past_key_values = None
        self._od.clear()
        self.used = 0
        if self.on_remove is not None:
            for node in nodes:
                self.on_remove(node)

    def nodes(self):
        return [node for node, _ in self._od.values()]

    def __len__(self):
        return len(self._od)
```

### genlm-backend_amd/sis.py

```python
import asyncio

import os

import numpy as np
import torch

from .cache import KVPrefix
from .engine import check_truncation
from .fuse import SplitConv1D, split_gemm_all_rows
from .kv import PACKED_MAX_KEYS, PrefixTable, PromptGroups, SlabKV, SlabRunner, encode_packed, encode_ragged, packed_supported
from ._lib import MASK_BITS, MASK_NONE
from .masks import ParticleMasks

RNG_PHILOX, RNG_NOISE = 1, 2


def make_masks(llm, max_token_length):
    eos_id = llm.tokenizer.eos_token_id
    V = len(llm.byte_vocab)
    valid = torch.tensor([tid == eos_id or len(tok) <= max_token_length for tid, tok in enumerate(llm.byte_vocab)],
                         dtype=torch.float).log()
    eos_one_hot = torch.nn.functional.one_hot(torch.tensor(eos_id), V).log()
    masks = torch.stack([valid, eos_one_hot.to(torch.float)])
    llm.register_masks(masks)
    return masks


def make_masking_function(llm, max_token_length, max_tokens):
    make_masks(llm, max_token_length)
    return lambda context: 1 if len(context) >= max_tokens else 0


class Particle:

    def __init__(self, llm, mask_selector, prompt_ids, eos_id):
        self.context = []
        self.prompt_ids = prompt_ids
        self.log_weight = 0.0
        self.active = True
        self.llm = llm
        self.mask_selector = mask_selector
        self.eos_id = eos_id

    async def extend(self):
        logZ, token = await self.llm.next_token_step(self.prompt_ids + self.context,
                                                     mask_id=self.mask_selector(self.context))
        self.log_weight += logZ
        if token == self.eos_id or token < 0:
            self.active = False
        else:
            self.context.append(token)


async def autobatched_sis(n_particles, llm, mask_selector, prompt_ids, eos_id, gather=None):
    gather = gather or asyncio.gather
    particles = [Particle(llm, mask_selector, prompt_ids, eos_id) for _ in range(n_particles)]
    while any(p.active for p in particles):
        await gather(*[p.extend() for p in particles if p.active])
    return particles


def _gather_all(dist, out, inp):
    if inp.is_cuda and dist.get_backend() == "gloo":
        host = torch.empty(out.shape, dtype=out.dtype)
        dist.all_gather_into_tensor(host, inp.cpu())
        out.copy_(host)
    else:
        dist.all_gather_into_tensor(out, inp)


def _all_to_all(dist, out, inp, out_splits, in_splits):
    if inp.is_cuda and dist.get_backend() == "gloo":
        host = torch.empty(out.shape, dtype=out.dtype)
        dist.all_to_all_single(host, inp.cpu(), output_split_sizes=out_splits, input_split_sizes=in_splits)
        out.copy_(host)
    else:
        dist.all_to_all_single(out, inp, output_split_sizes=out_splits, input_split_sizes=in_splits)


def _all_to_all_any(dist, out, inp, out_splits, in_splits):
    if inp.is_cuda and dist.get_backend() == "gloo":
        host = torch.empty(out.shape, dtype=out.dtype)
        dist.all_to_all_single(host, inp.cpu(), output_split_sizes=out_splits, input_split_sizes=in_splits)
        out.copy_(host)
    else:
        dist.all_to_all_single(out, inp, output_split_sizes=out_splits, input_split_sizes=in_splits)


def _reduce_all(dist, t, op):
    if t.is_cuda and dist.get_backend() == "gloo":
        host = t.cpu()
        dist.all_reduce(host, op=op)
        t.copy_(host)
    else:
        dist.all_reduce(t, op=op)


class CollectiveClock:

    def __init__(self):
        self.on = False
        self.events, self.host_s, self.calls, self.bytes = [], 0.0, 0, 0

    def start(self):
        self.on = True
        self.events, self.host_s, self.calls, self.bytes = [], 0.0, 0, 0

    def run(self, fn, tensor, nbytes):
        if not self.on:
            return fn()
        self.calls += 1
        self.bytes += int(nbytes)
        if tensor.is_cuda and self._device_timed:
            e0, e1 = torch.cuda.Event(enable_timing=True), torch.cuda.Event(enable_timing=True)
            e0.record()
            out = fn()
            e1.record()
            self.events.append((e0, e1))
            return out
        import time

        t0 = time.perf_counter()
        out = fn()
        self.host_s += time.perf_counter() - t0
        return out

    _device_timed = True

    def total_us(self):
        return self.host_s * 1e6 + sum(a.elapsed_time(b) for a, b in self.events) * 1e3


class DeviceSIS:

    def __init__(self, llm, n_particles, prompt_ids, max_tokens, eos_id, seed=0, rng="philox", rank=0, world=1,
                 dist=None, use_prefix_kv=False, use_particle_kv=False, resample_ess=None, force_collectives=False,
                 share_kv=True, kv_rows=None, kv_in_place=0.75, kv_graph=True, particle_masks=None, migrate_kv=True,
                 constraint=None, share_prompt_rows=True, proposal_temperature=None, proposal=None):
        if constraint is not None and particle_masks is not None:
            raise ValueError("give particle_masks (the caller's bit rows) or constraint (masks made on the device), not both")
        self._propose = proposal_temperature is not None or proposal is not None
        if self._propose:
            if rng != "philox":
                raise ValueError(f"proposal_temperature / proposal need rng='philox', got rng={rng!r}: the reference has no draw "
                                 "from a proposal for the parity mode to be on par with")
            if proposal_temperature is not None and not float(proposal_temperature) > 0.0:
                raise ValueError(f"proposal_temperature must be > 0, got {proposal_temperature!r}")
            if proposal is not None:
                for flag, name in ((use_prefix_kv, "use_prefix_kv"), (use_particle_kv, "use_particle_kv")):
                    if flag:
                        raise ValueError(f"proposal= conflicts with {name}: a proposal model is served on the re-encoding path "
                                         "only (it keeps no KV rows)")
                vp, vq = int(llm.model.config.vocab_size), int(proposal.model.config.vocab_size)
                if vp != vq:
                    raise ValueError(f"proposal= has another vocabulary: {vq} tokens, the target {vp}")
                if proposal.device != llm.device:
                    raise ValueError(f"proposal= is on {proposal.device}, the target on {llm.device}")
        self.proposal = proposal
        self._q_scale = 1.0 if proposal_temperature is None else 1.0 / float(proposal_temperature)
        self._q_logits = None
        self.constraint = constraint
        self.llm, self.eng, self.dev = llm, llm.engine, llm.device
        self._lora_epoch = getattr(llm, "lora_epoch", 0)
        if hasattr(llm, "_lora_sync"):
            llm._lora_sync(self._lora_epoch)
        self.N, self.max_tokens, self.eos_id = n_particles, max_tokens, eos_id
        self.rank, self.world, self.dist = rank, world, dist
        self.collective = world > 1 or (bool(force_collectives) and dist is not None)
        self.coll_clock = CollectiveClock()
        if dist is not None:
            self.coll_clock._device_timed = dist.get_backend() != "gloo"
        self.rows_moved_total = 0
        self.migrate_kv = bool(migrate_kv)
        self.kv_rows_moved = 0
        self.seed = seed
        self.rng_mode = RNG_PHILOX if rng == "philox" else RNG_NOISE
        self.noise_src = None
        self.noise_ahead = os.environ.get("GLB_RNG_AHEAD", "0") == "1"
        prompts = prompt_ids if isinstance(prompt_ids[0], (list, tuple)) else [prompt_ids] * n_particles
        assert len(prompts) == n_particles
        self._prompt_len0 = torch.tensor([len(p) for p in prompts], dtype=torch.int32, device=self.dev)
        self.max_prompt = max(len(p) for p in prompts)
        if self.collective:
            mp_ = torch.tensor([self.max_prompt], dtype=torch.int64, device=self.dev)
            _reduce_all(dist, mp_, dist.ReduceOp.MAX)
            self.max_prompt = int(mp_.item())
        lens = {len(p) for p in prompts}
        if self.collective and resample_ess is not None:
            mm = torch.tensor([min(lens), -max(lens)], dtype=torch.int64, device=self.dev)
            _reduce_all(dist, mm, dist.ReduceOp.MIN)
            lens = {int(mm[0]), int(-mm[1])}
        self._mask_by_row = len(lens) == 1
        self._rep = None
        self.cap = self.max_prompt + max_tokens + 1
        ctx = np.zeros((n_particles, self.cap), np.int32)
        for i, p in enumerate(prompts):
            ctx[i, :len(p)] = p
        self._ctx0 = torch.from_numpy(ctx).to(self.dev)
        self.starts = (torch.arange(n_particles, device=self.dev, dtype=torch.int64) * self.cap)
        self.prefixes = None
        if use_prefix_kv:
            distinct = {tuple(p) for p in prompts}
            if self.collective and resample_ess is not None:
                width = self.max_prompt
                all_p = torch.empty((world * n_particles, width), dtype=torch.int32, device=self.dev)
                all_l = torch.empty(world * n_particles, dtype=torch.int32, device=self.dev)
                _gather_all(dist, all_p.view(-1), self._ctx0[:, :width].contiguous().view(-1))
                _gather_all(dist, all_l, self._prompt_len0)
                all_p, all_l = all_p.cpu().numpy(), all_l.cpu().numpy()
                distinct = {tuple(int(t) for t in all_p[i, :all_l[i]]) for i in range(len(all_l))}
            self._build_prefixes(sorted(distinct))
        self.particle_kv = bool(use_particle_kv)
        self.share_kv = bool(share_kv) and self.particle_kv
        self.share_prompt_rows = bool(share_prompt_rows)
        self.packed_steps = 0
        self._groups = self._grp0 = None
        if self.share_prompt_rows and not use_prefix_kv and not use_particle_kv and not (self.collective and world > 1):
            index = {}
            grp = [index.setdefault(tuple(p), len(index)) for p in prompts]
            self._groups = PromptGroups(list(index), self.dev)
            self._grp0 = torch.tensor(grp, dtype=torch.int32, device=self.dev)
        self.kv_rows = int(kv_rows) if kv_rows is not None else n_particles
        self.kv_stats = dict(forward_rows=0, encoded_rows=0, copied_rows=0, unkept_rows=0, steps=0, in_place_steps=0)
        self._kv = SlabRunner(llm, self.kv_rows, self.cap, kv_in_place, kv_graph)
        if self.particle_kv:
            assert not use_prefix_kv
        self._particle = ParticleMasks(self.eng, n_particles, particle_masks)
        self.constraint_raw_steps = 0
        self.rows_moved = 0
        self.resample_ess = resample_ess
        self.n_resamples = 0
        self.sync_every = 1
        self.reset()

    pkv = property(lambda self: self._kv.pkv)
    particle_masks = property(lambda self: self._particle.masks, lambda self, masks: setattr(self._particle, "masks", masks))
    pm_raw_above = property(lambda self: self._particle.raw_above, lambda self, frac: setattr(self._particle, "raw_above", frac))
    pm_raw_steps = property(lambda self: self._particle.raw_steps)
    _slab_fwd = property(lambda self: self._kv._slab_fwd)

    @torch.no_grad()
    def _build_prefixes(self, distinct):
        llm, dev = self.llm, self.dev
        entries = []
        for p in distinct:
            out = llm._body(input_ids=torch.tensor([list(p)], device=dev), use_cache=True)
            entries.append((KVPrefix.from_hf_cache(out.past_key_values), p))
        self.prefixes = PrefixTable(entries, dev)

    def reset(self):
        if self.noise_src is not None:
            self.noise_src.reset()
        self._particle.reset()
        self.contexts = self._ctx0.clone()
        self.prompt_len = self._prompt_len0.clone()
        self._grp = self._grp0
        self.lengths = self.prompt_len.clone()
        self.active = torch.ones(self.N, dtype=torch.int32, device=self.dev)
        self.log_weights = torch.full((self.N,), getattr(self.constraint, "start_logw", 0.0), dtype=torch.float32, device=self.dev)
        self.states =self.constraint.states0(self.N) if self.constraint is not None else None
        self.t = 0
        self.max_len_now = self.max_prompt
        self.last_stats = None
        self.kernel_events = []
        self.outer_events = []
        self._event_pool = []
        self._head_cache = None
        self._noise_buf = getattr(self, "_noise_buf", None)
        self._fwd_tokens = None
        self._noise_groups = None
        self._kv_stale = None
        self._row_of_d = torch.full((self.N,), -1, dtype=torch.int32, device=self.dev)
        self._global_active = torch.tensor(self.N * self.world, dtype=torch.int32, device=self.dev)
        self.all_weights = None
        self._all_stamp = None
        self._rehash()

    def _rehash(self):
        ctx_flat = self.contexts.view(-1)
        self.hashes = self.eng.hash_contexts(ctx_flat, self.starts, self.lengths)
        self._hash_stub = self.eng.hash_contexts(ctx_flat, self.starts, torch.ones_like(self.lengths))

    @torch.no_grad()
    def _encode_into_slabs(self, rows):
        eng, llm, dev, N = self.eng, self.llm, self.dev, self.N
        ctx_flat = self.contexts.view(-1)
        kv_len = self.lengths if self.t == 0 else (self.lengths - 1).clamp_min(1)
        want = torch.ones(N, dtype=torch.bool, device=dev) if rows is None else \
            torch.zeros(N, dtype=torch.bool, device=dev).index_fill_(0, rows, True)
        lens_eff = torch.where(want, kv_len, torch.ones_like(kv_len))
        group_of, rep, ng = eng.group_contexts(ctx_flat, self.starts, lens_eff)
        U = int(ng.item())
        l_max = int(lens_eff.max().item())
        enc = encode_ragged(llm, (ctx_flat, self.starts, lens_eff), rep, U, l_max, keep_kv=True)
        src = enc.kv_layers()
        if self.pkv is None:
            self._kv.pkv = SlabKV(eng, N, self.cap, len(src))
        src_row = torch.where(want, group_of, torch.full_like(group_of, -1))
        self.pkv.fill_rows(src, src_row, lens_eff)
        return enc, group_of, rep, U

    @torch.no_grad()
    def _step_particle_kv(self, time_kernel):
        eng, llm, dev, N = self.eng, self.llm, self.dev, self.N
        if self.t % self.sync_every == 0 or self._head_cache is None:
            head = torch.stack([self.active.sum().to(torch.int32), self._global_active, eng.error_word()[0]]).cpu()
            eng.raise_if_failed(int(head[2]))
            self._head_cache = (int(head[0]), int(head[1]))
        n_active, n_global = self._head_cache
        if self._kv_stale is not None:
            self._encode_into_slabs(torch.nonzero(self._kv_stale).flatten())
            self._kv_stale = None
        rows = torch.arange(N, device=dev)
        pos = (self.lengths - 1).clamp_min(0)
        newest = self.contexts[rows, pos.long()]
        ids = torch.where(self.active > 0, newest, torch.zeros_like(newest)).view(N, 1).long()
        logits = llm._lm_head(self._kv.slab_forward()(ids, pos))
        self._noise_groups = None
        if self.rng_mode == RNG_NOISE:
            lengths_eff = torch.where(self.active > 0, self.lengths, torch.ones_like(self.lengths))
            self._noise_groups, _, _ = eng.group_contexts(self.contexts.view(-1), self.starts, lengths_eff)
        return self._finish_step(logits, None, N, n_active, n_global, time_kernel, l_max=1)

    @torch.no_grad()
    def _step_shared_kv(self, time_kernel):
        eng, N, R = self.eng, self.N, self.kv_rows
        ctx_flat = self.contexts.view(-1)
        lengths_eff = torch.where(self.active > 0, self.lengths, torch.ones_like(self.lengths))
        hashes_eff = torch.where(self.active > 0, self.hashes, self._hash_stub)
        group_of, rep, ng = eng.group_contexts(ctx_flat, self.starts, lengths_eff, hashes=hashes_eff)
        plan = eng.kv_plan(group_of, rep, ng, self._row_of_d, lengths_eff, R, self.cap, by_context=True)
        head = torch.cat([plan["head"][:6], torch.stack([self.active.sum().to(torch.int32), self._global_active,
                                                          eng.error_word()[0]])]).cpu().tolist()
        U, nA, nB, n_copied, n_unkept, l_max_b, n_active, n_global = head[:8]
        eng.raise_if_failed(head[8])
        self._row_of_d = plan["row_of_context"]
        st = self.kv_stats
        st["forward_rows"] += U
        st["encoded_rows"] += nB
        st["copied_rows"] += n_copied
        st["unkept_rows"] += n_unkept
        st["steps"] += 1
        logits, self._fwd_tokens, in_place = self._kv.run(plan, head[:6], lambda ctx, pos: self.contexts[ctx, pos],
                                                          (ctx_flat, self.starts, lengths_eff))
        st["in_place_steps"] += int(in_place)
        self._rep = torch.cat([plan["ctx_a"][:nA], plan["ctx_b"][:nB]])
        self._noise_groups = group_of
        row_of = plan["logits_row"][group_of.long()]
        return self._finish_step(logits, row_of, U, n_active, n_global, time_kernel, l_max=1)

    def _finish_step(self, logits, group_of, U, n_active, n_global, time_kernel, l_max):
        eng, llm, N = self.eng, self.llm, self.N
        V = logits.shape[-1]
        mask_id = ((self.lengths - self.prompt_len) >= self.max_tokens).to(torch.int32)
        if self._propose:
            return self._finish_proposed(logits, group_of, U, n_active, n_global, time_kernel, l_max, mask_id)
        source = self.constraint if self.constraint is not None else self._particle if self.particle_masks is not None else llm.masks
        kw, raw = source.step_masks(logits, *self._mask_units(logits, group_of, mask_id), N, parity=self.rng_mode == RNG_NOISE)
        self.constraint_raw_steps += int(raw and self.constraint is not None)
        if self.rng_mode == RNG_NOISE:
            kw["noise"] = self._parity_noise(self._noise_groups if self._noise_groups is not None else group_of, V)
        if time_kernel:
            if len(self._event_pool) < 2:
                self._event_pool = eng.timing_events(64)
            inner, (e0, e1) = self._event_pool.pop(), self._event_pool.pop()
            e0.record()
            kw["timing_events"] = inner
        logZ, _, tok = eng.step(logits, vocab=V, row_of=group_of, rng_mode=self.rng_mode, seed=self.seed,
                                offset=self.t, particle_base=self.rank * N, want_lse=False, **kw)
        if time_kernel:
            e1.record()
            self.kernel_events.append(inner)
            self.outer_events.append((e0, e1))
        if self.rng_mode == RNG_NOISE:
            self.noise_src.prefetch()
        return self._advance(logits, mask_id, logZ, tok, U, n_active, n_global, l_max)

    def _proposal_masks(self, logits, ids, by_row):
        key = "row_mask_id" if by_row else "mask_id"
        if self.constraint is not None:
            kw, raw = self.constraint.step_masks(logits, ids, by_row, self.N, parity=False)
            self.constraint_raw_steps += int(raw)
            return kw
        if self.particle_masks is not None:
            return {"mask_kind": MASK_BITS, "mask": self.particle_masks, key: ids}
        m = self.llm.masks
        return {} if m.kind == MASK_NONE else {"mask_kind": m.kind, "mask": m.table, key: ids}

    def _finish_proposed(self, logits, group_of, U, n_active, n_global, time_kernel, l_max, mask_id):
        eng, N = self.eng, self.N
        kw = self._proposal_masks(logits, *self._mask_units(logits, group_of, mask_id))
        q, self._q_logits = self._q_logits, None
        if time_kernel:
            if len(self._event_pool) < 2:
                self._event_pool = eng.timing_events(64)
            e0, e1 = self._event_pool.pop()
            e0.record()
        dlogw, tok, _ = eng.importance_step(logits, q, proposal_scale=self._q_scale, vocab=logits.shape[-1], row_of=group_of,
                                            seed=self.seed, offset=self.t, particle_base=self.rank * N, **kw)
        if time_kernel:
            e1.record()
            self.kernel_events.append((e0, e1))
            self.outer_events.append((e0, e1))
        return self._advance(logits, mask_id, dlogw, tok, U, n_active, n_global, l_max)

    def _advance(self, logits, mask_id, logZ, tok, U, n_active, n_global, l_max):
        eng = self.eng
        len_was = self.lengths.clone() if self.constraint is not None else None
        if self.constraint is not None and self.constraint.weighted:
            self.log_weights += self.constraint.forced_final_logw(self.states, (mask_id > 0) & (self.active > 0) & (tok == self.eos_id))
        eng.particles_advance(self.contexts, self.lengths, self.active, self.log_weights, logZ, tok, self.eos_id,
                              self.cap, hashes=self.hashes)
        if self.constraint is not None:
            self.constraint.advance(self.states, self.contexts, len_was, self.lengths, out=self.states)
        self.t += 1
        self.max_len_now = min(self.max_len_now + 1, self.cap)
        ft = self._fwd_tokens if self._fwd_tokens is not None else U * l_max
        self._fwd_tokens = None
        self.last_stats = dict(n_unique=U, n_active=n_active, l_max=l_max, n_rows=U, fwd_tokens=ft, head_rows=logits.shape[0])
        self._exchange()
        if self.resample_ess is not None:
            self._maybe_resample()
        return U, n_global

    def _mask_units(self, logits, group_of, done):
        if self.constraint is None and self.particle_masks is not None:
            own = torch.arange(self.N, dtype=torch.int32, device=self.dev)
            return torch.where(done > 0, torch.full_like(own, self.N), own), False
        ids = done if self.constraint is None else self.constraint.mask_rows(self.states, done=done)
        if self._mask_by_row and group_of is not None:
            ids = ids[self._rep[:logits.shape[0]].long()].contiguous()
        return ids, self._mask_by_row

    def _recompute_states(self):
        if self.constraint is not None:
            self.states = self.constraint.advance(None, self.contexts, self.prompt_len, self.lengths)

    def update_particle_masks(self, rows, bit_rows):
        self._particle.update(rows, bit_rows)

    def _exchange(self):
        count = self.active.sum().to(torch.float32).view(1)
        if self.collective:
            N = self.N
            parts = [self.log_weights, count]
            carry = self.rng_mode == RNG_NOISE and self.world > 1
            if carry:
                parts += [self.hashes.view(torch.float32), self.active.to(torch.float32)]
            mine = torch.cat(parts)
            out = torch.empty((self.world, mine.numel()), dtype=torch.float32, device=self.dev)
            self.coll_clock.run(lambda: _gather_all(self.dist, out.view(-1), mine), mine, out.numel() * 4)
            self.all_weights = out[:, :N].reshape(-1)
            self._global_active = out[:, N].sum().to(torch.int32)
            if carry:
                self._all_hashes = out[:, N + 1:3 * N + 1].contiguous().view(torch.int64).reshape(-1)
                self._all_active = out[:, 3 * N + 1:].reshape(-1) > 0
                self._all_stamp = (self.t, self.n_resamples)
        else:
            self.all_weights = self.log_weights
            self._global_active = count[0].to(torch.int32)

    @torch.no_grad()
    def step(self, time_kernel=False):
        eng, llm, dev, N = self.eng, self.llm, self.dev, self.N
        if hasattr(llm, "_lora_sync"):
            llm._lora_sync(self._lora_epoch)
        if self.share_kv:
            return self._step_shared_kv(time_kernel)
        if self.particle_kv and self.t > 0:
            return self._step_particle_kv(time_kernel)
        ctx_flat = self.contexts.view(-1)
        lengths_eff = torch.where(self.active > 0, self.lengths, torch.ones_like(self.lengths))
        if self.particle_kv:
            head = torch.stack([self.active.sum().to(torch.int32), self._global_active, eng.error_word()[0]]).cpu()
            n_active, n_global = int(head[0]), int(head[1])
            eng.raise_if_failed(int(head[2]))
            enc, group_of, rep, U = self._encode_into_slabs(None)
            self._rep = rep
            self._noise_groups = None
            return self._finish_step(llm._lm_head(enc.last_rows()), group_of, U, n_active, n_global, time_kernel, self.max_len_now)
        hashes_eff = torch.where(self.active > 0, self.hashes, self._hash_stub)
        group_of, rep, ng = eng.group_contexts(ctx_flat, self.starts, lengths_eff, hashes=hashes_eff)
        self._rep = rep
        head = torch.stack([ng[0], self.active.sum().to(torch.int32), self._global_active, eng.error_word()[0]]).cpu()
        U, n_active, n_global = int(head[0]), int(head[1]), int(head[2])
        eng.raise_if_failed(int(head[3]))
        base, prefixes = None, None
        l_max = self.max_len_now
        if self.prefixes is not None and self.t > 0:
            P = self.prefixes
            pref, base = eng.match_prefixes(ctx_flat, self.starts, lengths_eff, P.tokens, P.starts, P.lengths)
            prefixes = (P, pref[rep[:U].long()].contiguous())
            l_max = max(self.t, 1)
        if self._packed_ready(U, n_active, l_max):
            with split_gemm_all_rows(eng):
                enc = encode_packed(llm, (ctx_flat, self.starts, lengths_eff), rep, U, self._grp[rep[:U].long()],
                                    self._groups, U * self.t, max_keys=l_max)
            self._fwd_tokens = enc.n_rows
            self.packed_steps += 1
        else:
            enc = encode_ragged(llm, (ctx_flat, self.starts, lengths_eff), rep, U, l_max, base=base, prefixes=prefixes)
        logits = llm._lm_head(enc.last_rows())
        if self.proposal is not None:
            other = self.proposal
            self._q_logits = other._lm_head(encode_ragged(other, (ctx_flat, self.starts, lengths_eff), rep, U, l_max).last_rows())
        self._noise_groups = None
        return self._finish_step(logits, group_of, U, n_active, n_global, time_kernel, l_max)

    def _packed_ready(self, U, n_active, l_max):
        if self._groups is None or self.t < 1 or n_active != self.N or l_max > PACKED_MAX_KEYS or self.prefixes is not None:
            return False
        body = self.llm._body
        ent = self.__dict__.get("_packed_body")
        if ent is None or ent[0] is not body:
            rows = [m.min_rows for m in body.modules() if isinstance(m, SplitConv1D)]
            ent = self._packed_body = (body, max(rows) if rows and packed_supported(self.llm) else None)
        return ent[1] is not None and U * l_max >= ent[1]

    def _parity_noise(self, group_of, V):
        N = self.N
        if self.noise_src is None:
            self.noise_src = self.eng.noise_rng(self.seed, V, ahead=self.noise_ahead and self.world == 1)
        if self.collective and self.world > 1:
            return self._parity_noise_sharded(V)
        act = self.active > 0
        key = torch.where(act, group_of.to(torch.int64), torch.full((N,), 1 << 40, dtype=torch.int64, device=self.dev))
        order = torch.argsort(key, stable=True)
        rank = torch.empty(N, dtype=torch.int32, device=self.dev)
        rank[order] = torch.arange(N, dtype=torch.int32, device=self.dev)
        slot = torch.where(act, rank, torch.full_like(rank, -1))
        if self._noise_buf is None or self._noise_buf.shape != (N, V):
            self._noise_buf = torch.empty((N, V), dtype=torch.float32, device=self.dev)
        return self.noise_src.rows(N, row_slot=slot, n_draw=act.sum().to(torch.int32), max_draw=N, out=self._noise_buf)

    def _parity_noise_sharded(self, V):
        N, dev = self.N, self.dev
        if getattr(self, "_all_stamp", None) != (self.t, self.n_resamples):
            mine = torch.cat([self.hashes.view(torch.float32), self.active.to(torch.float32)])
            out = torch.empty((self.world, 3 * N), dtype=torch.float32, device=dev)
            self.coll_clock.run(lambda: _gather_all(self.dist, out.view(-1), mine), mine, out.numel() * 4)
            self._all_hashes = out[:, :2 * N].contiguous().view(torch.int64).reshape(-1)
            self._all_active = out[:, 2 * N:].reshape(-1) > 0
            self._all_stamp = (self.t, self.n_resamples)
        h, act = self._all_hashes, self._all_active
        NT = h.numel()
        ar = torch.arange(NT, device=dev)
        sh, perm = torch.sort(h, stable=True)
        start = torch.ones(NT, dtype=torch.bool, device=dev)
        start[1:] = sh[1:] != sh[:-1]
        first = perm[torch.cummax(torch.where(start, ar, torch.zeros_like(ar)), 0).values]
        key = torch.empty(NT, dtype=torch.int64, device=dev)
        key[perm] = first
        key = torch.where(act, key, torch.full_like(key, 1 << 40))
        order = torch.argsort(key, stable=True)
        place = torch.empty(NT, dtype=torch.int32, device=dev)
        place[order] = torch.arange(NT, dtype=torch.int32, device=dev)
        slot = torch.where(act, place, torch.full_like(place, -1))[self.rank * N:(self.rank + 1) * N].contiguous()
        if self._noise_buf is None or self._noise_buf.shape != (N, V):
            self._noise_buf = torch.empty((N, V), dtype=torch.float32, device=dev)
        return self.noise_src.rows(N, row_slot=slot, n_draw=act.sum().to(torch.int32), max_draw=NT, out=self._noise_buf)

    def gather_weights(self):
        if self.all_weights is None:
            self._exchange()
        return self.all_weights

    def normalized_weights(self):
        return self.eng.normalize_weights(self.gather_weights())

    @torch.no_grad()
    def _maybe_resample(self):
        n_total = self.N * self.world
        if self.resample_ess < 1.0:
            _, stats = self.eng.normalize_weights(self.all_weights)
            if float(stats[1].item()) >= self.resample_ess * n_total:
                return
        self.resample()

    @torch.no_grad()
    def resample(self):
        eng, N, dev = self.eng, self.N, self.dev
        n_total = N * self.world
        anc, lse = eng.resample_systematic(self.all_weights, self.seed ^ 0x5eed5a11, self.t)
        mine = anc[self.rank * N:(self.rank + 1) * N].contiguous()
        state = torch.cat([self.contexts, torch.stack([self.lengths, self.prompt_len, self.active], dim=1)], dim=1).contiguous()
        local = mine - self.rank * N
        new_state = eng.gather_rows_i32(state, local.clamp(0, N - 1))
        if self.collective and self.world > 1:
            anc_h = anc.cpu().numpy()
            owner = anc_h // N
            r = self.rank
            send_idx = [anc_h[d * N:(d + 1) * N][owner[d * N:(d + 1) * N] == r] - r * N if d != r else anc_h[:0]
                        for d in range(self.world)]
            mine_owner = owner[r * N:(r + 1) * N]
            recv_cnt = [int((mine_owner == src).sum()) if src != r else 0 for src in range(self.world)]
            self.rows_moved = int((owner != np.repeat(np.arange(self.world), N)).sum())
            self.rows_moved_total += self.rows_moved
            moved = None
            if self.rows_moved:
                take = np.concatenate(send_idx).astype(np.int64)
                take_d = torch.from_numpy(take).to(dev)
                send = state[take_d] if len(take) else state[:0]
                recv = torch.empty((sum(recv_cnt), state.shape[1]), dtype=torch.int32, device=dev)
                send_cnt = [len(x) for x in send_idx]
                send = send.contiguous()
                self.coll_clock.run(lambda: _all_to_all(self.dist, recv, send, recv_cnt, send_cnt), send,
                                    (send.numel() + recv.numel()) * 4)
                slots_d = None
                if sum(recv_cnt):
                    slots = np.concatenate([np.nonzero(mine_owner == src)[0] for src in range(self.world) if src != r])
                    slots_d = torch.from_numpy(slots.astype(np.int64)).to(dev)
                    new_state[slots_d] = recv
                moved = (take_d, send_cnt, slots_d, recv_cnt)
        self.contexts = new_state[:, :self.cap].contiguous()
        self.lengths, self.prompt_len, self.active = (new_state[:, self.cap + k].contiguous() for k in range(3))
        self.log_weights = (lse - float(np.log(n_total))).expand(N).contiguous()
        if self._grp is not None:
            self._grp = self._grp[local.clamp(0, N - 1).long()]
        if self.share_kv:
            local = mine - self.rank * N
            ok = (local >= 0) & (local < N)
            self._row_of_d = torch.where(ok, self._row_of_d[local.clamp(0, N - 1).long()], torch.full_like(local, -1))
        elif self.particle_kv and self.pkv is not None:
            local = mine - self.rank * N
            is_local = (local >= 0) & (local < N)
            src = torch.where(is_local, local, torch.full_like(local, -1))
            kv_len = (self.lengths - 1).clamp_min(0)
            self.pkv.gather(src, kv_len)
            stale = ~is_local
            if self.migrate_kv and self.collective and self.world > 1:
                if self.rows_moved:
                    self._migrate_kv(*moved)
                self._kv_stale = None
            else:
                self._kv_stale = stale if bool(stale.any().item()) else None
        self._rehash()
        self._recompute_states()
        self.n_resamples += 1
        self._exchange()

    def _migrate_kv(self, take_d, send_cnt, slots_d, recv_cnt):
        pkv = self.pkv
        new = pkv._tensors(pkv.layers)
        old = pkv._alt
        n_send, n_recv = int(sum(send_cnt)), int(sum(recv_cnt))
        shape = tuple(new[0].shape[1:])
        for t in new:
            if tuple(t.shape[1:]) != shape or t.dtype != new[0].dtype:
                raise ValueError("KV layers of different shapes: rows cannot travel in one message")
        send = torch.stack([t[take_d] for t in old], dim=1).contiguous() if n_send else new[0].new_zeros((0, len(new)) + shape)
        recv = new[0].new_empty((n_recv, len(new)) + shape)
        self.coll_clock.run(lambda: _all_to_all_any(self.dist, recv, send, recv_cnt, send_cnt), send,
                            (send.numel() + recv.numel()) * send.element_size())
        if n_recv:
            for j, t in enumerate(new):
                t[slots_d] = recv[:, j]
        self.kv_rows_moved += n_recv

    @torch.no_grad()
    def run(self, max_steps=None):
        steps = 0
        limit = max_steps if max_steps is not None else self.max_tokens + 1
        while steps < limit:
            _, n_global = self.step()
            steps += 1
            if n_global == 0:
                break
        return steps

    @torch.no_grad()
    def rescore(self, llm=None, prompt_ids=None, constraint=None):
        llm = self.llm if llm is None else llm
        gen = self.lengths - self.prompt_len
        drew_eos = (self.active == 0) & torch.isfinite(self.log_weights) & (self.lengths < self.cap)
        at_end = self.lengths.clamp(max=self.cap - 1).long()[:, None]
        last = torch.where(drew_eos[:, None], torch.full_like(at_end, self.eos_id), self.contexts.gather(1, at_end))
        tokens = self.contexts.scatter(1, at_end, last.to(torch.int32))
        lengths, plen = self.lengths + drew_eos.to(torch.int32), self.prompt_len
        forced_at = None
        if constraint is not None:
            forced_at = torch.where(drew_eos & (gen >= self.max_tokens), gen, torch.full_like(gen, -1))
        if prompt_ids is not None:
            prompt = torch.tensor(list(prompt_ids), dtype=torch.int32, device=self.dev)
            if prompt.numel() == 0:
                raise ValueError("a prompt needs at least one token")
            n_p = prompt.numel()
            j = torch.arange(n_p + self.cap, device=self.dev)[None] - n_p
            own = torch.gather(tokens, 1, (plen[:, None].long() + j).clamp(0, self.cap - 1))
            shared = prompt[(j + n_p).clamp(min=0, max=n_p - 1)].expand(self.N, -1)
            tokens = torch.where(j < 0, shared, own).contiguous()
            plen = torch.full_like(plen, n_p)
            lengths = plen + gen + drew_eos.to(torch.int32)
        return llm.batch_sequence_logprobs_device(tokens, lengths, plen, constraint=constraint, forced_at=forced_at)

    def results(self):
        self.eng.check()
        if self.constraint is not None:
            self.constraint.check()
        ctx = self.contexts.cpu().numpy()
        ln = self.lengths.cpu().numpy()
        pl = self.prompt_len.cpu().numpy()
        return [list(ctx[i, pl[i]:ln[i]]) for i in range(self.N)], self.log_weights.cpu().numpy()


class DeviceSampler(DeviceSIS):

    def __init__(self, llm, prompts, max_tokens, eos_token_ids, temperature=1.0, seed=None, sync_every=4, top_k=0, top_p=1.0,
                 min_p=0.0):
        top_k, top_p, log_min_p = check_truncation(top_k, top_p, min_p)
        super().__init__(llm, len(prompts), [list(p) for p in prompts], max_tokens, eos_id=-1,
                         seed=0 if seed is None else int(seed), rng="philox", use_particle_kv=True, share_kv=False,
                         kv_graph=max_tokens >= 64)
        self.sync_every = max(1, int(sync_every))
        self.temperature = float(temperature)
        self.truncation = dict(top_k=top_k, top_p=top_p, min_p=float(min_p))
        self.truncated = top_k > 0 or top_p < 1.0 or log_min_p > float("-inf")
        self._row_ids = None
        self.eos = torch.tensor(sorted(set(int(t) for t in eos_token_ids)), dtype=torch.int32, device=self.dev)
        self.seeded = seed is not None
        if not self.seeded:
            self.seed = int(torch.randint(0, 2**62, (1,)).item())

    def _finish_step(self, logits, group_of, U, n_active, n_global, time_kernel, l_max):
        eng, N, dev = self.eng, self.N, self.dev
        V = logits.shape[-1]
        kw = {}
        mode = RNG_PHILOX
        if self.seeded:
            mode = RNG_NOISE
            if self.noise_src is None:
                self.noise_src = eng.noise_rng(self.seed, V)
            kw["noise"] = self.noise_src.rows(1)
        if self.truncated:
            bits = eng.truncate_rows(logits, vocab=V, logit_scale=1.0 / self.temperature, **self.truncation)["bits"]
            if self._row_ids is None or self._row_ids.numel() != bits.shape[0]:
                self._row_ids = torch.arange(bits.shape[0], dtype=torch.int32, device=dev)
            kw.update(mask_kind=MASK_BITS, mask=bits, row_mask_id=self._row_ids)
        _, _, tok = eng.step(logits, vocab=V, row_of=group_of, rng_mode=mode, seed=self.seed, offset=self.t,
                             logit_scale=1.0 / self.temperature, want_lse=False, **kw)
        act = (self.active > 0) & (tok != -2)
        stop = act & (torch.isin(tok, self.eos) | (tok < 0) | (self.lengths - self.prompt_len >= self.max_tokens))
        keep = act & ~stop
        rows = torch.arange(N, device=dev)
        at = self.lengths.long().clamp_max(self.cap - 1)
        self.contexts[rows, at] = torch.where(keep, tok, self.contexts[rows, at])
        self.lengths = self.lengths + keep.to(torch.int32)
        self.active = torch.where(tok == -2, self.active, (keep & (self.lengths - self.prompt_len < self.max_tokens)).to(torch.int32))
        self.t += 1
        self.max_len_now = min(self.max_len_now + 1, self.cap)
        self._exchange()
        return U, n_global

    def generate(self):
        steps = 0
        while steps < self.max_tokens:
            _, n_global = self.step()
            steps += 1
            if n_global == 0:
                break
        return self.results()[0]


class SisBenchWorkload:

    def __init__(self, eng, dev, rank, world, dist, n_particles=1024, max_tokens=10, prefix_kv=False, particle_kv=False,
                 model="gpt2", n_prompts=1, resample=False, force_collectives=False, kv_in_place=0.75,
                 per_particle_masks=False, rng="philox", gemms="library", share_prompt_rows=True):
        from .llm import AsyncAmdLM

        if model == "gpt2":
            from transformers import GPT2Config

            cfg, dtype = GPT2Config(), torch.float32
            self.model_name = "gpt2-small shape (random init, fp32)"
        elif model == "llama-3-8b":
            from transformers import LlamaConfig

            cfg = LlamaConfig(vocab_size=128256, hidden_size=4096, intermediate_size=14336, num_hidden_layers=32,
                              num_attention_heads=32, num_key_value_heads=8, head_dim=128, max_position_embeddings=4096,
                              rope_theta=500000.0, rms_norm_eps=1e-5, tie_word_embeddings=False, bos_token_id=128000,
                              eos_token_id=128001)
            dtype = torch.bfloat16
            self.model_name = "Llama-3-8B shape (random init, bf16)"
        else:
            from transformers import LlamaConfig

            cfg = LlamaConfig(vocab_size=128256, hidden_size=2048, intermediate_size=8192, num_hidden_layers=16,
                              num_attention_heads=32, num_key_value_heads=8, head_dim=64, max_position_embeddings=4096,
                              rope_theta=500000.0, rms_norm_eps=1e-5, tie_word_embeddings=True, bos_token_id=128000,
                              eos_token_id=128001)
            dtype = torch.bfloat16
            self.model_name = "Llama-3.2-1B shape (random init, bf16)"
        self.dtype_name = "f32" if dtype == torch.float32 else "bf16"
        self.elem = 4 if dtype == torch.float32 else 2
        self.llm = AsyncAmdLM.from_config(cfg, None, device=dev, dtype=dtype, seed=1234, engine=eng,
                                          batch_size=n_particles, gemms=gemms)
        V = cfg.vocab_size
        g = torch.Generator(device=dev)
        g.manual_seed(4321)
        valid = torch.where(torch.rand(V, device=dev, generator=g) < 1 / 3, float("-inf"), 0.0)
        valid[cfg.eos_token_id] = 0.0
        eos1 = torch.full((V,), float("-inf"), device=dev)
        eos1[cfg.eos_token_id] = 0.0
        self.llm.register_masks(torch.stack([valid, eos1]))
        pm = None
        if per_particle_masks:
            own = torch.where(torch.rand((n_particles, V), device=dev, generator=g) < 1 / 3, float("-inf"), 0.0)
            own[:, cfg.eos_token_id] = 0.0
            pm, _ = eng.mask_to_bits(torch.cat([own, eos1[None]]))
            del own
        self.per_particle_masks = per_particle_masks
        self.V, self.N, self.max_tokens = V, n_particles, max_tokens
        self.particles_per_step = n_particles
        rs = np.random.default_rng(99)
        base = [list(range(100, 108))] + [[int(t) for t in rs.integers(1000, 30000, 8)] for _ in range(n_prompts - 1)]
        prompts = [base[i % n_prompts] for i in range(n_particles)] if n_prompts > 1 else base[0]
        self.n_prompts = n_prompts
        self.rng = rng
        self.sis = DeviceSIS(self.llm, n_particles, prompts, max_tokens, cfg.eos_token_id,
                             seed=1234, rng=rng, rank=rank, world=world, dist=dist, use_prefix_kv=prefix_kv,
                             use_particle_kv=particle_kv, resample_ess=1.0 if resample else None,
                             force_collectives=force_collectives, kv_in_place=kv_in_place, particle_masks=pm,
                             share_prompt_rows=share_prompt_rows)
        self.prefix_kv = prefix_kv
        self.particle_kv = particle_kv
        self.resample = resample
        self.kernel_bytes = None
        self._events = []
        self._outer = []
        self._bytes = []
        self.unique_hist = []
        self.fed_hist = []
        self.flops_hist = []
        body = self.llm._body
        self._lin_w = sum(m.weight.numel() for m in body.modules() if type(m).__name__ in ("Linear", "Conv1D", "SplitConv1D"))
        self._lin_w += sum(m.in_features * m.out_features for m in body.modules() if type(m).__name__ == "W4Linear")
        self._head_w = self.llm._head.weight.numel()
        for _ in range(max_tokens):
            self.sis.step(time_kernel=False)
        self.sis.reset()
        torch.cuda.synchronize(dev)

    def step(self, i, timed):
        if self.sis.t >= self.max_tokens:
            self._collect()
            self.sis.reset()
        U, _ = self.sis.step(time_kernel=timed)
        if timed:
            n_masks = self.N + 1 if self.per_particle_masks else 2
            self._bytes.append(U * self.V * self.elem + n_masks * ((self.V + 31) // 32) * 4 + self.N * 8
                               + (self.N * self.V * 4 if self.rng != "philox" else 0))
            self.unique_hist.append(U)
            self.fed_hist.append(int(self.sis.last_stats["l_max"]))
            ls = self.sis.last_stats
            self.flops_hist.append(2.0 * self._lin_w * ls["fwd_tokens"] + 2.0 * self._head_w * ls["head_rows"])

    def _collect(self):
        self._events.extend(self.sis.kernel_events)
        self._outer.extend(self.sis.outer_events)
        self.sis.kernel_events = []
        self.sis.outer_events = []

    def kernel_times_us(self):
        self._collect()
        self.kernel_bytes = float(np.mean(self._bytes)) if self._bytes else 0.0
        self.kernel_bytes_each = np.array(self._bytes, dtype=np.float64)
        return np.array([a.elapsed_time(b) * 1e3 for a, b in self._events])

    def keep_kernel_times(self, n):
        self._collect()
        for name in ("_events", "_outer", "_bytes", "unique_hist", "fed_hist", "flops_hist"):
            setattr(self, name, getattr(self, name)[:n])

    def outer_times_us(self):
        return np.array([a.elapsed_time(b) * 1e3 for a, b in self._outer])

    def config(self):
        return {"workload": f"SIS step: {self.N} particles/GPU, {self.model_name}, prompt len 8, <=10 new "
                            "tokens, " + (f"{self.N} per-particle bit masks (standing still: handed over raw at the first step, prepared from the second on)" if self.per_particle_masks
                                          else "2 shared bit masks") + ", device-resident population, "
                            + ("Philox draws" if self.rng == "philox" else "the reference's draws (torch.multinomial's CPU MT19937 stream, "
                               "generated on the device: ids identical to torch's under the seed)")
                            + (f", {self.n_prompts} distinct shared prompts" if self.n_prompts > 1 else "")
                            + (", prompt KV cached (cache_kv semantics, BASELINE config 3)" if self.prefix_kv else "")
                            + (", device-resident KV rows shared by particles with equal contexts (one new token per distinct "
                               "context per step; NOT the reference's re-encode-every-step algorithm)" if self.particle_kv else "")
                            + (", systematic resampling after every step" if self.resample else ""),
                "particles_per_gpu": self.N, "vocab": self.V,
                "rng": "philox" if self.rng == "philox" else "parity (torch CPU generator on the device)",
                "mean_unique_contexts_per_step": float(np.mean(self.unique_hist)) if self.unique_hist else None,
                "mean_tokens_fed_per_context": float(np.mean(self.fed_hist)) if self.fed_hist else None,
                "gemm_flops_per_step": float(np.mean(self.flops_hist)) if self.flops_hist else None,
                **({"prefixed_tokens_per_context": 8} if self.prefix_kv else {}),
                **({"kv_rows": {k: v for k, v in self.sis.kv_stats.items()}} if self.particle_kv else {})}
```

### include/glb.h

```cpp
#ifndef GLB_H
#define GLB_H

#include <stddef.h>
#include <stdint.h>

#ifdef __cplusplus
extern "C" {
#endif

#define GLB_ABI_VERSION 9

enum {
  GLB_OK = 0,
  GLB_EINVAL = 1,
  GLB_EUNSUPPORTED = 2,
  GLB_EHIP = 3,
  GLB_ENOSPC = 4
};

enum { GLB_F32 = 0, GLB_BF16 = 1, GLB_F16 = 2 };

enum {
  GLB_MASK_NONE = 0,
  GLB_MASK_BITS = 1,
// ... 90 lines not shown

int glb_gather_kv_padded(const void *const *slabs, const int32_t *slab_len, int64_t n_prefixes,
                         const int32_t *prefix_of, int64_t n_rows, int64_t heads,
                         int64_t head_dim, int64_t p_max, int32_t elem_bytes, void *out,
                         void *hip_stream);

int glb_particles_advance(int32_t *contexts, int64_t ctx_ld, int32_t *lengths, int32_t *active,
                          float *log_weights, const float *logZ, const int32_t *token, int64_t n,
                          int32_t eos_id, int32_t max_len, uint64_t *ctx_hashes, void *hip_stream);

int glb_normalize_weights(const float *log_weights, int64_t n, float *out_probs, float *out_stats,
                          void *hip_stream);

int glb_kv_append(void *slab, const void *new_rows, const int32_t *pos, const int32_t *row_of, int64_t n_rows,
                  int64_t heads, int64_t cap, int64_t head_dim, int64_t new_stride_row, int64_t new_stride_head,
                  int32_t elem_bytes, void *hip_stream);
int glb_kv_gather_rows(const void *const *src, void *const *dst, int64_t n_tensors, int64_t n_rows, int64_t heads,
                       int64_t head_dim, int64_t src_cap, int64_t dst_cap, const int32_t *src_row_of,
                       const int32_t *len_of, int32_t elem_bytes, void *hip_stream);
int glb_gather_rows_i32(const int32_t *src, int64_t src_ld, const int32_t *row_of, int64_t n, int64_t width,
                        int32_t *dst, int64_t dst_ld, void *hip_stream);

int glb_match_rows(const int32_t *tokens, const int64_t *starts, const int32_t *lengths, const int32_t *rep,
                   const int32_t *n_groups, int64_t n, const int32_t *row_tok, const int32_t *row_len,
                   const uint64_t *row_hash, int64_t n_rows, int64_t cap, int32_t *out_old_row, uint64_t *out_hash,
                   void *hip_stream);
typedef struct glb_kv_plan_args {
  uint32_t struct_size;
  int64_t n, n_rows, cap;
  const int32_t *group_of, *rep, *n_groups;
  const int32_t *old_row;
  int32_t old_row_by_context;
  const int32_t *lengths;
  int64_t *row_stamps;
  int64_t call_no;
  int32_t *row_tok, *row_len;
  uint64_t *row_hash;
  const uint64_t *group_hash;
  const int32_t *tokens;
  const int64_t *starts;
  int32_t *out_group_row, *out_logits_row, *out_rows_a, *out_ctx_a, *out_pos_a, *out_ctx_b, *out_rows_b, *out_copy_src,
      *out_copy_len, *out_ctx_of_row, *out_pos_of_row, *out_row_of_context, *out_head;
  void *workspace;
  size_t workspace_bytes;
} glb_kv_plan_args;
size_t glb_kv_plan_workspace(int64_t n, int64_t n_rows);
int glb_kv_plan(const glb_kv_plan_args *args, void *hip_stream);

#define GLB_KV_CHUNK_MAX 16
int glb_match_prefix_rows(const int32_t *tokens, const int64_t *starts, const int32_t *lengths, const int32_t *rep,
                          const int32_t *n_groups, int64_t n, const int32_t *row_tok, const int32_t *row_len,
                          const uint64_t *row_hash, int64_t n_rows, int64_t cap, int32_t max_new, int32_t *out_old_row,
                          int32_t *out_keep, uint64_t *out_hash, void *hip_stream);
typedef struct glb_kv_plan_chunk_args {
  uint32_t struct_size;
  glb_kv_plan_args plan;
  const int32_t *old_keep;
  int32_t *out_n_new_a, *out_n_new_of_row;
} glb_kv_plan_chunk_args;
int glb_kv_plan_chunk(const glb_kv_plan_chunk_args *args, void *hip_stream);
int glb_slab_attention_chunk(const void *q, const int64_t q_strides[3], const void *k_new, const int64_t k_strides[3],
                             const void *v_new, const int64_t v_strides[3], void *k_slab, void *v_slab, const int32_t *pos,
                             const int32_t *n_new, const int32_t *row_of, int64_t n_rows, int64_t n_slab_rows, int64_t heads,
                             int64_t kv_heads, int64_t cap, int64_t head_dim, int64_t max_new, float scale, int32_t dtype,
                             void *out, void *hip_stream);

int glb_slab_attention(const void *q, int64_t q_stride_row, int64_t q_stride_head, const void *k_new, int64_t k_stride_row,
                       int64_t k_stride_head, const void *v_new, int64_t v_stride_row, int64_t v_stride_head, void *k_slab,
                       void *v_slab, const int32_t *pos,
                       int64_t n_rows, int64_t heads, int64_t kv_heads, int64_t cap, int64_t head_dim, float scale,
                       int32_t dtype, void *out, void *hip_stream);

int glb_short_attention(const void *q, const int64_t q_strides[3], const void *k, const int64_t k_strides[3], const void *v,
                        const int64_t v_strides[3], const uint8_t *mask, int64_t mask_stride_row, int64_t mask_stride_query,
                        int64_t n_rows, int64_t heads, int64_t kv_heads, int64_t q_len, int64_t k_len, int64_t head_dim,
                        float scale, int32_t dtype, void *out, void *hip_stream);

int glb_short_attention_packed(const void *q, int64_t q_stride_row, int64_t q_stride_head, const void *k, int64_t k_stride_row,
                               int64_t k_stride_head, const void *v, int64_t v_stride_row, int64_t v_stride_head,
                               const int32_t *plan, int64_t n_segments, int64_t n_rows, int64_t heads, int64_t kv_heads,
                               int64_t max_keys, int64_t head_dim, float scale, int32_t dtype, void *out, uint32_t *err_word,
                               void *hip_stream);

size_t glb_resample_workspace(int64_t n);
int glb_resample_systematic(const float *log_weights, int64_t n, uint64_t seed, uint64_t offset,
                            int32_t *out_ancestors, float *out_stats, void *workspace, size_t workspace_bytes,
                            void *hip_stream);

enum { GLB_TRIE_SUM = 0, GLB_TRIE_MAX = 1 };
size_t glb_trie_workspace(int64_t n_rows, int64_t n_nodes);
int glb_trie_reduce(const float *weights, int64_t ld, int64_t n_rows, int64_t vocab, int64_t n_nodes, int64_t n_levels,
                    const int32_t *leaf_node, const int32_t *level_start_host, const int32_t *level_nodes,
                    const int32_t *child_ptr, const int32_t *child_idx, int32_t op, int32_t from_logprobs, float *out,
                    int64_t out_ld, void *workspace, size_t workspace_bytes, void *hip_stream);

typedef struct glb_trie_args {
  uint32_t struct_size;
  const void *weights;
  int32_t dtype;
  int64_t ld, n_rows, vocab;
  const float *lse;
  float logit_scale;
  int32_t from_logprobs;
  int32_t op;
  int64_t n_nodes, n_levels;
  const int32_t *leaf_node, *level_start_host, *level_nodes, *child_ptr, *child_idx;
  float *out;
  int64_t out_ld;
  const int32_t *sel_nodes;
  int64_t n_sel;
  float *out_sel;
  int64_t out_sel_ld;
  int32_t keep_node_major;
  void *workspace;
  size_t workspace_bytes;
} glb_trie_args;
size_t glb_trie_workspace_ex(int64_t n_rows, int64_t n_nodes);
int glb_trie_masses(const glb_trie_args *args, void *hip_stream);

typedef struct glb_trie_plan {
  uint32_t struct_size;
  int32_t n_parts, n_top, n_cut, n_slots, max_local, top_base, lds_bytes;
  int64_t n_nodes;
  const int32_t *desc, *idepth, *leaf_src, *leaf_local, *run_tab, *top_local, *slot_of;
  const uint16_t *cptr16, *inode16, *pn_local16;
  const uint16_t *tok_local16;
  const uint64_t *inode64;
  int32_t lds_top_bytes, vocab;
} glb_trie_plan;
typedef struct glb_trie_rows_args {
  uint32_t struct_size;
  const void *weights;
  int32_t dtype;
  int64_t ld, n_rows, vocab;
  const float *lse;
  float logit_scale;
  int32_t from_logprobs;
  int32_t op;
  float *out_slots;
  int64_t out_slots_ld;
  float *out_nodes;
  int64_t out_nodes_ld;
  const int32_t *sel_nodes;
  int64_t n_sel;
  float *out_sel;
  int64_t out_sel_ld;
  void *workspace;
  size_t workspace_bytes;
  int64_t sel_row_stride;
} glb_trie_rows_args;
size_t glb_trie_rows_workspace(int64_t n_rows, const glb_trie_plan *plan);
int glb_trie_rows(const glb_trie_rows_args *args, const glb_trie_plan *plan, void *hip_stream);

typedef struct glb_mt19937 {
  uint32_t mt[624];
  int32_t idx;
} glb_mt19937;
void glb_mt19937_seed(glb_mt19937 *st, uint64_t seed);
int glb_mt19937_exponential_f32(glb_mt19937 *st, float *out, int64_t n);

#define GLB_MT_POLY_WORDS 312
int glb_mt19937_window(uint64_t seed, uint32_t *out_window );
int glb_mt19937_jump_polys(int64_t stride_words, int32_t n_small, int32_t n_big, uint64_t *out_polys );
int glb_mt19937_jump_host(const uint32_t *window_in, const uint64_t *poly, uint32_t *window_out);
typedef struct glb_mt_rows_args {
  uint32_t struct_size;
  const uint32_t *window;
  uint32_t *window_out;
  const uint64_t *polys;
  int32_t n_small, n_big;
  int64_t vocab;
  int64_t max_draw_rows;
  const int32_t *n_draw;
  int64_t n_out_rows;
  const int32_t *row_slot;
  float *out;
  int64_t out_ld;
  void *workspace;
  size_t workspace_bytes;
  int32_t reuse_windows;
  const float *rows_from;
  int64_t rows_from_ld;
} glb_mt_rows_args;
size_t glb_mt19937_rows_workspace(int64_t max_draw_rows, int32_t n_small);
int glb_mt19937_exponential_rows(const glb_mt_rows_args *args, void *hip_stream);

#define GLB_COMM_ID_BYTES 128
int glb_comm_unique_id(void *out_id);
int glb_comm_init(const void *id, int32_t rank, int32_t world, void **out_comm);
int glb_allgather_f32(void *comm, const float *send, int64_t n, float *recv, void *hip_stream);
int glb_comm_destroy(void *comm);

enum { GLB_GEMM_BIAS = 0, GLB_GEMM_BIAS_GELU_TANH = 1 };
typedef struct glb_gemm_args {
  uint32_t struct_size;
  int64_t m, n, k;
  const float *a;
  int64_t lda;
  const void *w_split;
  const float *bias;
  float *c;
  int64_t ldc;
  int32_t epilogue;
} glb_gemm_args;
size_t glb_gemm_split_bytes(int64_t k, int64_t n);
int glb_gemm_split_weights(const float *w, int64_t k, int64_t n, int64_t ldw, void *out, size_t out_bytes, void *hip_stream);
int glb_gemm_f32_split(const glb_gemm_args *args, void *hip_stream);
enum { GLB_GEMM_FORM_LARGE = 1, GLB_GEMM_FORM_SMALL = 2 };
int glb_gemm_split_pick(int64_t m, int64_t n, int64_t k, int n_cus, int *form);
int glb_gemm_f32_split_form(const glb_gemm_args *args, int form, void *hip_stream);
int glb_gemm_f32_split_residual(const glb_gemm_args *args, const float *residual, int64_t ldr, int form, void *hip_stream);
int glb_gemm_split_blocks_per_cu(int gelu, int *blocks);
int glb_gemm_split_form_blocks_per_cu(int form, int gelu, int *blocks);

typedef struct glb_packed_plan_args {
  uint32_t struct_size;
  int64_t n_tokens, n_contexts, n_sel, n_groups, n_pre, n_tail_rows, pos_cap;
  const int32_t *tokens;
  const int64_t *starts;
  const int32_t *lengths;
  const int32_t *sel;
  const int32_t *grp;
  const int32_t *group_starts;
  const int32_t *group_lens;
  const int32_t *group_segments;
  const int64_t *group_ids;
  const int64_t *group_pos;
  int32_t *segments;
  int64_t *ids;
  int64_t *pos;
  int64_t *last;
  int32_t *ends;
} glb_packed_plan_args;
int glb_packed_plan(const glb_packed_plan_args *args, void *hip_stream);

typedef struct glb_lora_job {
  uint32_t struct_size;
  int32_t w_dtype;
  int32_t ab_dtype;
  int32_t w_transposed;
  int64_t n_out, k_in, r;
  const void *w;
  int64_t ldw;
  const void *a;
  int64_t lda;
  const void *b;
  int64_t ldb;
  float scale;
  void *out;
  int64_t ldo;
} glb_lora_job;
size_t glb_lora_merge_workspace_bytes(int32_t n_jobs);
int glb_lora_merge(const glb_lora_job *jobs , int32_t n_jobs, void *workspace , size_t workspace_bytes,
                   void *hip_stream);

typedef struct glb_lora_rows_entry {
  uint32_t struct_size;
  int32_t ab_dtype;
  int64_t n_out, k_in, r;
  const void *a;
  int64_t lda;
  const void *b;
  int64_t ldb;
  float scale;
} glb_lora_rows_entry;
typedef struct glb_lora_rows_args {
  uint32_t struct_size;
  int32_t dtype;
  int64_t m, n, k;
  const void *x;
  int64_t ldx;
  void *y;
  int64_t ldy;
  const void *row_slot;
  const void *table;
  int32_t n_slots, n_modules;
  int32_t module;
  int32_t r_max;
  void *workspace;
  size_t workspace_bytes;
} glb_lora_rows_args;
size_t glb_lora_rows_table_bytes(int32_t n_slots, int32_t n_modules);
int glb_lora_rows_table_upload(const glb_lora_rows_entry *entries , int32_t n_slots, int32_t n_modules,
                               void *table , size_t table_bytes, void *hip_stream);
size_t glb_lora_rows_workspace_bytes(int64_t m, int32_t r_max);
int glb_lora_rows(const glb_lora_rows_args *args, void *hip_stream);

typedef struct glb_w4_args {
  uint32_t struct_size;
  int32_t dtype;
  int32_t transposed;
  int64_t n, k;
  void *w;
  int64_t ldw;
  const float *codebook;
  void *image;
  size_t image_bytes;
} glb_w4_args;
typedef struct glb_w4_gemm_args {
  uint32_t struct_size;
  int32_t dtype;
  int64_t m, n, k;
  const void *x;
  int64_t ldx;
  const void *image;
  const float *codebook;
  const void *bias;
  void *y;
  int64_t ldy;
  void *workspace;
  size_t workspace_bytes;
} glb_w4_gemm_args;
size_t glb_w4_bytes(int64_t n, int64_t k);
int glb_w4_quantize(const glb_w4_args *args, void *hip_stream);
int glb_w4_dequantize(const glb_w4_args *args, void *hip_stream);
int glb_w4_gemm_max_rows(void);
size_t glb_w4_gemm_workspace_bytes(int64_t m, int64_t n, int64_t k);
// ... 417 lines not shown
```

Baseline: 146,300.

## Plan packed forward on device with fixed-size slots to avoid host syncs

Adds a device-side packed plan that gives every particle a fixed-size slot of rows. Dead slots are zero-filled by the attention kernel, so the step no longer needs to read unique counts back to the host before building the packed batch. The SIS step gains a lagged, sync-free mode that uses earlier head results, and benchmark byte counts are resolved lazily. The cost is extra padded rows of compute and a dense fallback whenever the slot conditions fail.

```diff
diff --git a/genlm-backend_amd/_lib.py b/genlm-backend_amd/_lib.py
--- a/genlm-backend_amd/_lib.py
+++ b/genlm-backend_amd/_lib.py
@@ -197,6 +197,20 @@
         ("group_starts", C.c_void_p), ("group_lens", C.c_void_p), ("group_segments", C.c_void_p),
         ("group_ids", C.c_void_p), ("group_pos", C.c_void_p),
         ("segments", C.c_void_p), ("ids", C.c_void_p), ("pos", C.c_void_p), ("last", C.c_void_p), ("ends", C.c_void_p),
+    ]
+
+
+class PackedPlanSlotsArgs(C.Structure):
+    _fields_ = [
+        ("struct_size", C.c_uint32),
+        ("n_tokens", C.c_int64), ("n_contexts", C.c_int64), ("n_groups", C.c_int64), ("n_pre", C.c_int64),
+        ("slot_rows", C.c_int64), ("pos_cap", C.c_int64),
+        ("tokens", C.c_void_p), ("starts", C.c_void_p), ("lengths", C.c_void_p), ("active", C.c_void_p),
+        ("group_of", C.c_void_p), ("rep", C.c_void_p), ("n_groups_found", C.c_void_p), ("grp", C.c_void_p),
+        ("group_starts", C.c_void_p), ("group_lens", C.c_void_p), ("group_segments", C.c_void_p),
+        ("group_ids", C.c_void_p), ("group_pos", C.c_void_p),
+        ("segments", C.c_void_p), ("ids", C.c_void_p), ("pos", C.c_void_p), ("last", C.c_void_p), ("row_of", C.c_void_p),
+        ("live_count", C.c_void_p),
     ]
 
 
@@ -577,6 +591,8 @@
                                       _i64, _i64, _i64, _i64, _i64, _i64, _f32, _i32, _vp, _vp]),
     "glb_short_attention_packed": (C.c_int, [_vp, _i64, _i64, _vp, _i64, _i64, _vp, _i64, _i64, _vp, _i64, _i64, _i64, _i64, _i64,
                                              _i64, _f32, _i32, _vp, _vp, _vp]),
+    "glb_short_attention_packed_slots": (C.c_int, [_vp, _i64, _i64, _vp, _i64, _i64, _vp, _i64, _i64, _vp, _i64, _i64, _i64, _i64,
+                                                   _i64, _i64, _f32, _i32, _i64, _vp, _vp, _vp]),
     "glb_kv_plan_workspace": (_sz, [_i64, _i64]),
     "glb_kv_plan": (C.c_int, [C.POINTER(KvPlanArgs), _vp]),
     "glb_match_prefix_rows": (C.c_int, [_vp, _vp, _vp, _vp, _vp, _i64, _vp, _vp, _vp, _i64, _i64, _i32, _vp, _vp, _vp, _vp]),
@@ -610,6 +626,7 @@
     "glb_gemm_f32_split_form": (C.c_int, [C.POINTER(GemmArgs), C.c_int, _vp]),
     "glb_gemm_f32_split_residual": (C.c_int, [C.POINTER(GemmArgs), _vp, _i64, C.c_int, _vp]),
     "glb_packed_plan": (C.c_int, [C.POINTER(PackedPlanArgs), _vp]),
+    "glb_packed_plan_slots": (C.c_int, [C.POINTER(PackedPlanSlotsArgs), _vp]),
     "glb_gemm_split_blocks_per_cu": (C.c_int, [C.c_int, C.POINTER(C.c_int)]),
     "glb_gemm_split_form_blocks_per_cu": (C.c_int, [C.c_int, C.c_int, C.POINTER(C.c_int)]),
     "glb_lora_merge_workspace_bytes": (_sz, [_i32]),
diff --git a/genlm-backend_amd/csrc/glb_kv.hip b/genlm-backend_amd/csrc/glb_kv.hip
--- a/genlm-backend_amd/csrc/glb_kv.hip
+++ b/genlm-backend_amd/csrc/glb_kv.hip
@@ -823,6 +823,7 @@
   int64_t q_sr, q_sh, k_sr, k_sh, v_sr, v_sh;
   int32_t S, M, H, Hkv, max_keys;
   float scale;
+  int32_t zero_tail;
 };
 
 template <int DT, int DH, int KMAX>
@@ -838,6 +839,18 @@
   const int32_t *seg = a.plan + (int64_t)s * 4;
   const int64_t pre_start = seg[0], pre_len = seg[1], tail_start = seg[2], tail_len = seg[3];
   const int64_t n_keys = pre_len + tail_len;
+  if (a.zero_tail > 0 && tail_len == 0) {
+    if (tail_start < 0 || tail_start + a.zero_tail > a.M) {
+      if (lane == 0 && hk == 0) atomicAdd(a.err, 1u);
+      return;
+    }
+    const int per_row = G * LP;
+    for (int r = 0; r < a.zero_tail; ++r) {
+      char *row = a.out + ((tail_start + r) * a.H + (int64_t)hk * G) * DH * ES;
+      for (int c = lane; c < per_row; c += 64) *reinterpret_cast<u32x4 *>(row + (int64_t)c * 16) = u32x4{0u, 0u, 0u, 0u};
+    }
+    return;
+  }
   if (pre_len < 0 || tail_len < 1 || n_keys > a.max_keys || n_keys > KMAX || pre_start < 0 || pre_start + pre_len > a.M ||
       tail_start < 0 || tail_start + tail_len > a.M) {
     if (lane == 0 && hk == 0) atomicAdd(a.err, 1u);
@@ -1323,6 +1336,18 @@
                                const int32_t *plan, int64_t n_segments, int64_t n_rows, int64_t heads, int64_t kv_heads,
                                int64_t max_keys, int64_t head_dim, float scale, int32_t dtype, void *out, uint32_t *err_word,
                                void *stream) {
+  return glb_short_attention_packed_slots(q, q_stride_row, q_stride_head, k, k_stride_row, k_stride_head, v, v_stride_row,
+                                          v_stride_head, plan, n_segments, n_rows, heads, kv_heads, max_keys, head_dim, scale,
+                                          dtype, 0, out, err_word, stream);
+}
+
+int glb_short_attention_packed_slots(const void *q, int64_t q_stride_row, int64_t q_stride_head, const void *k,
+                                     int64_t k_stride_row, int64_t k_stride_head, const void *v, int64_t v_stride_row,
+                                     int64_t v_stride_head, const int32_t *plan, int64_t n_segments, int64_t n_rows,
+                                     int64_t heads, int64_t kv_heads, int64_t max_keys, int64_t head_dim, float scale,
+                                     int32_t dtype, int64_t zero_tail_rows, void *out, uint32_t *err_word, void *stream) {
+  if (zero_tail_rows < 0 || zero_tail_rows > 0x7fffffffll)
+    return glb::api_fail(GLB_EINVAL, "glb_short_attention_packed_slots: %lld rows per dead slot", (long long)zero_tail_rows);
   if (!q || !k || !v || !out || !plan || !err_word) return glb::api_fail(GLB_EINVAL, "glb_short_attention_packed: null pointer");
   if (dtype < GLB_F32 || dtype > GLB_F16) return glb::api_fail(GLB_EINVAL, "bad dtype %d", dtype);
   if (n_segments <= 0 || n_rows <= 0 || heads <= 0 || kv_heads <= 0 || heads % kv_heads || heads > 0x7fffffffll ||
@@ -1353,6 +1378,7 @@
   a.Hkv = (int32_t)kv_heads;
   a.max_keys = (int32_t)max_keys;
   a.scale = scale;
+  a.zero_tail = (int32_t)zero_tail_rows;
   hipError_t e;
   switch (dtype) {
     case GLB_F32: e = launch_short_packed<GLB_F32>(a, (int)head_dim, (hipStream_t)stream); break;
diff --git a/genlm-backend_amd/csrc/glb_packed_plan.hip b/genlm-backend_amd/csrc/glb_packed_plan.hip
--- a/genlm-backend_amd/csrc/glb_packed_plan.hip
+++ b/genlm-backend_amd/csrc/glb_packed_plan.hip
@@ -88,6 +88,100 @@
   a.pos[row] = p < 0 ? 0 : (p > a.pos_cap - 1 ? a.pos_cap - 1 : p);
 }
 
+struct Slot {
+  bool live, refused;
+  int32_t pre_start, pre_len, rep;
+};
+
+__device__ __forceinline__ Slot read_slot(const glb_packed_plan_slots_args &a, int64_t i) {
+  const int64_t N = a.n_contexts, G = a.n_groups;
+  int64_t ng = a.n_groups_found[0];
+  ng = ng < 1 ? 1 : (ng > N ? N : ng);
+  int64_t g = a.group_of[i];
+  g = g < 0 ? 0 : (g > ng - 1 ? ng - 1 : g);
+  int64_t p = a.grp[i];
+  p = p < 0 ? 0 : (p > G - 1 ? G - 1 : p);
+  Slot s;
+  s.rep = a.rep[g];
+  s.pre_start = a.group_starts[p];
+  s.pre_len = a.group_lens[p];
+  const bool mine = a.active[i] > 0 && (int64_t)s.rep == i;
+  s.live = mine && a.lengths[i] == wrap_add(s.pre_len, (int32_t)a.slot_rows);
+  s.refused = mine && !s.live;
+  return s;
+}
+
+__global__ __launch_bounds__(ROW_THREADS) void packed_plan_slots_kernel(glb_packed_plan_slots_args a) {
+  __shared__ int32_t wave_sum[ROW_THREADS / 64];
+  const int64_t row = (int64_t)blockIdx.x * ROW_THREADS + threadIdx.x;
+  const int64_t N = a.n_contexts, T = a.slot_rows, M = a.n_pre + N * T;
+  if (row < a.n_groups * 4) a.segments[row] = a.group_segments[row];
+  if (row < a.n_pre) {
+    a.ids[row] = a.group_ids[row];
+    a.pos[row] = a.group_pos[row];
+  } else if (row < M) {
+    const int64_t r = row - a.n_pre, i = r / T, j = r - i * T;
+    const Slot s = read_slot(a, i);
+    int64_t id = 0, p = 0;
+    if (s.live) {
+      const int32_t pos_t = wrap_add(s.pre_len, (int32_t)j);
+      int64_t at = a.starts[i] + (int64_t)pos_t;
+      at = at < 0 ? 0 : (at > a.n_tokens - 1 ? a.n_tokens - 1 : at);
+      id = (int64_t)a.tokens[at];
+      p = pos_t;
+      p = p < 0 ? 0 : (p > a.pos_cap - 1 ? a.pos_cap - 1 : p);
+    }
+    a.ids[row] = id;
+    a.pos[row] = p;
+    if (j == 0) {
+      int32_t *seg = a.segments + (a.n_groups + i) * 4;
+      seg[0] = s.pre_start;
+      seg[1] = s.pre_len;
+      seg[2] = (int32_t)row;
+      seg[3] = s.live ? (int32_t)T : (s.refused ? -1 : 0);
+      a.last[i] = s.live ? row + T - 1 : row;
+      const int64_t to = a.active[i] > 0 ? (int64_t)s.rep : i;
+      a.row_of[i] = (int32_t)(to < 0 ? 0 : (to > N - 1 ? N - 1 : to));
+    }
+  }
+  if (blockIdx.x != 0) return;
+  int32_t n = 0;
+  for (int64_t i = threadIdx.x; i < N; i += ROW_THREADS) n += read_slot(a, i).live ? 1 : 0;
+#pragma unroll
+  for (int d = 32; d >= 1; d >>= 1) n += __shfl_down(n, d, 64);
+  if ((threadIdx.x & 63) == 0) wave_sum[threadIdx.x >> 6] = n;
+  __syncthreads();
+  if (threadIdx.x == 0) {
+    int32_t total = 0;
+    for (int w = 0; w < ROW_THREADS / 64; ++w) total += wave_sum[w];
+    a.live_count[0] = total;
+  }
+}
+
+}
+
+extern "C" int glb_packed_plan_slots(const glb_packed_plan_slots_args *args, void *stream) {
+  if (!args) return glb::api_fail(GLB_EINVAL, "glb_packed_plan_slots: null argument block");
+  if (args->struct_size != sizeof(glb_packed_plan_slots_args))
+    return glb::api_fail(GLB_EINVAL, "glb_packed_plan_slots_args.struct_size %u != %zu (ABI mismatch)", args->struct_size,
+                         sizeof(glb_packed_plan_slots_args));
+  const glb_packed_plan_slots_args &a = *args;
+  if (a.n_groups < 1 || a.n_pre < 1 || a.slot_rows < 1 || a.n_contexts < 1 || a.n_tokens < 1 || a.pos_cap < 1 ||
+      a.n_groups > INT32_MAX / 4 || a.n_pre > INT32_MAX || a.slot_rows > INT32_MAX || a.n_contexts > INT32_MAX ||
+      a.n_pre + a.n_contexts * a.slot_rows > INT32_MAX)
+    return glb::api_fail(GLB_EINVAL, "glb_packed_plan_slots: bad sizes (G %lld, prompt rows %lld, %lld slots of %lld rows, tokens "
+                         "%lld, position cap %lld)", (long long)a.n_groups, (long long)a.n_pre, (long long)a.n_contexts,
+                         (long long)a.slot_rows, (long long)a.n_tokens, (long long)a.pos_cap);
+  if (!a.tokens || !a.starts || !a.lengths || !a.active || !a.group_of || !a.rep || !a.n_groups_found || !a.grp ||
+      !a.group_starts || !a.group_lens || !a.group_segments || !a.group_ids || !a.group_pos)
+    return glb::api_fail(GLB_EINVAL, "glb_packed_plan_slots: null input");
+  if (!a.segments || !a.ids || !a.pos || !a.last || !a.row_of || !a.live_count)
+    return glb::api_fail(GLB_EINVAL, "glb_packed_plan_slots: null output");
+  const int64_t M = a.n_pre + a.n_contexts * a.slot_rows, threads = M > a.n_groups * 4 ? M : a.n_groups * 4;
+  hipLaunchKernelGGL(packed_plan_slots_kernel, dim3(blocks_for(threads, ROW_THREADS)), dim3(ROW_THREADS), 0, (hipStream_t)stream, a);
+  const hipError_t e = hipGetLastError();
+  if (e != hipSuccess) return glb::api_hip_fail(e, "glb_packed_plan_slots launch");
+  return GLB_OK;
 }
 
 extern "C" int glb_packed_plan(const glb_packed_plan_args *args, void *stream) {
diff --git a/genlm-backend_amd/engine.py b/genlm-backend_amd/engine.py
--- a/genlm-backend_amd/engine.py
+++ b/genlm-backend_amd/engine.py
@@ -905,6 +905,35 @@
         check(self.lib.glb_packed_plan(C.byref(a), self._stream()))
         return seg, ids, pos, last
 
+    def packed_plan_slots(self, batch, active, group_of, rep, ng, grp, groups, slot_rows, pos_cap):
+        tokens, starts, lengths = batch
+        G, n_pre, N = len(groups.lens), groups.n_rows, lengths.numel()
+        ins = (tokens, starts, lengths, active, group_of, rep, ng, grp, groups.starts_d, groups.lens_d, groups.segments,
+               groups.ids, groups.pos)
+        self._check_dev(*ins)
+        want = (torch.int32, torch.int64) + (torch.int32,) * 9 + (torch.int64, torch.int64)
+        if any(t.dtype != d for t, d in zip(ins, want)):
+            raise ValueError(f"packed_plan_slots: dtypes {[t.dtype for t in ins]}, expected {list(want)}")
+        if any(t.numel() != N for t in (starts, active, group_of, rep, grp)) or ng.numel() < 1 or groups.ids.numel() != n_pre:
+            raise ValueError("packed_plan_slots: starts / lengths / active / group_of / rep / grp disagree, or the prompts' rows do")
+        if int(slot_rows) < 1:
+            raise ValueError("packed_plan_slots: a slot holds at least one row")
+        M = n_pre + N * int(slot_rows)
+        seg = torch.empty((G + N, 4), dtype=torch.int32, device=self.device)
+        ids = torch.empty(M, dtype=torch.int64, device=self.device)
+        pos = torch.empty(M, dtype=torch.int64, device=self.device)
+        last = torch.empty(N, dtype=torch.int64, device=self.device)
+        row_of, live = self._i32(N), self._i32(1)
+        a = _lib.PackedPlanSlotsArgs()
+        a.struct_size = C.sizeof(_lib.PackedPlanSlotsArgs)
+        a.n_tokens, a.n_contexts, a.n_groups, a.n_pre = tokens.numel(), N, G, n_pre
+        a.slot_rows, a.pos_cap = int(slot_rows), int(pos_cap)
+        (a.tokens, a.starts, a.lengths, a.active, a.group_of, a.rep, a.n_groups_found, a.grp, a.group_starts, a.group_lens,
+         a.group_segments, a.group_ids, a.group_pos) = (t.data_ptr() for t in ins)
+        a.segments, a.ids, a.pos, a.last, a.row_of, a.live_count = (t.data_ptr() for t in (seg, ids, pos, last, row_of, live))
+        check(self.lib.glb_packed_plan_slots(C.byref(a), self._stream()))
+        return seg, ids, pos, last, row_of, live
+
     def lora_merge(self, jobs):
         n = len(jobs)
         if n == 0:
@@ -1185,7 +1214,7 @@
                                            _DT[query.dtype], _ptr(out), self._stream()))
         return out
 
-    def short_attention_packed(self, query, key, value, plan, max_keys, scale, err=None, out=None):
+    def short_attention_packed(self, query, key, value, plan, max_keys, scale, err=None, out=None, zero_tail_rows=0):
         M, H, Dh = query.shape
         Hkv = key.shape[1]
         assert key.shape == value.shape == (M, Hkv, Dh) and key.dtype == value.dtype == query.dtype
@@ -1197,6 +1226,13 @@
         if out is None:
             out = torch.empty((M, H, Dh), dtype=query.dtype, device=self.device)
         assert out.shape == (M, H, Dh) and out.dtype == query.dtype and out.device == self.device and out.is_contiguous()
+        if zero_tail_rows:
+            check(self.lib.glb_short_attention_packed_slots(_ptr(query), query.stride(0), query.stride(1), _ptr(key), key.stride(0),
+                                                            key.stride(1), _ptr(value), value.stride(0), value.stride(1),
+                                                            _ptr(plan), plan.shape[0], M, H, Hkv, int(max_keys), Dh, float(scale),
+                                                            _DT[query.dtype], int(zero_tail_rows), _ptr(out), _ptr(err),
+                                                            self._stream()))
+            return out
         check(self.lib.glb_short_attention_packed(_ptr(query), query.stride(0), query.stride(1), _ptr(key), key.stride(0),
                                                   key.stride(1), _ptr(value), value.stride(0), value.stride(1), _ptr(plan),
                                                   plan.shape[0], M, H, Hkv, int(max_keys), Dh, float(scale),
diff --git a/genlm-backend_amd/kv.py b/genlm-backend_amd/kv.py
--- a/genlm-backend_amd/kv.py
+++ b/genlm-backend_amd/kv.py
@@ -38,7 +38,7 @@
             raise RuntimeError("glb_short_attention_packed: the attention module changed the shape of the packed batch")
         scale = scaling if scaling is not None else query.shape[-1] ** -0.5
         out = packed.engine.short_attention_packed(query[0].transpose(0, 1), key[0].transpose(0, 1), value[0].transpose(0, 1),
-                                                   packed.segments, packed.max_keys, scale)
+                                                   packed.segments, packed.max_keys, scale, zero_tail_rows=packed.zero_tail_rows)
         packed.served += 1
         return out.unsqueeze(0), None
     eng = getattr(getattr(module, "config", None), "_glb_engine", None)
@@ -596,8 +596,9 @@
 
 class PackedKV(Cache):
 
-    def __init__(self, engine, segments, n_rows, max_keys, n_layers):
+    def __init__(self, engine, segments, n_rows, max_keys, n_layers, zero_tail_rows=0):
         self.engine, self.segments, self.n_rows, self.max_keys = engine, segments, int(n_rows), int(max_keys)
+        self.zero_tail_rows = int(zero_tail_rows)
         self.served = 0
         layer = _PackedLayer(self)
         super().__init__(layers=[layer] * n_layers)
@@ -665,6 +666,46 @@
     return PackedEncoding(out, last, M)
 
 
+def packed_plan_slots(group_lens, grp, lens, active, group_of, rep, ng, t):
+    group_lens, grp, lens = np.asarray(group_lens, np.int64), np.asarray(grp, np.int64), np.asarray(lens, np.int64)
+    active, group_of, rep = np.asarray(active), np.asarray(group_of, np.int64), np.asarray(rep, np.int64)
+    N = len(lens)
+    g_start = np.concatenate([[0], np.cumsum(group_lens[:-1])])
+    n_pre = int(group_lens.sum())
+    to = rep[group_of.clip(0, min(max(int(ng), 1), N) - 1)]
+    mine = (active > 0) & (to == np.arange(N))
+    live = mine & (lens == group_lens[grp] + t)
+    start = n_pre + np.arange(N) * t
+    tail = np.where(live, t, np.where(mine, -1, 0))
+    zero = np.zeros_like(group_lens)
+    seg = np.concatenate([np.stack([zero, zero, g_start, group_lens], 1),
+                          np.stack([g_start[grp], group_lens[grp], start, tail], 1)]).astype(np.int32)
+    row_of = np.where(active > 0, to.clip(0, N - 1), np.arange(N)).astype(np.int32)
+    return seg, np.where(live, start + t - 1, start).astype(np.int64), row_of, int(live.sum())
+
+
+def encode_packed_slots(llm, batch, active, group_of, rep, ng, grp, groups, t, max_keys=PACKED_MAX_KEYS):
+    eng = llm.engine
+    if not 1 <= max_keys <= PACKED_MAX_KEYS:
+        raise ValueError(f"encode_packed_slots serves contexts of up to {PACKED_MAX_KEYS} tokens")
+    if t < 1:
+        raise ValueError("encode_packed_slots: every slot feeds at least one row")
+    if not packed_supported(llm):
+        raise RuntimeError("encode_packed_slots: this model's attention is not served by glb_short_attention")
+    max_pos = getattr(llm._body.config, "max_position_embeddings", None) or (1 << 30)
+    segments, ids, pos, last, row_of, live = eng.packed_plan_slots(batch, active, group_of, rep, ng, grp, groups, t,
+                                                                   min(PACKED_MAX_KEYS, max_pos))
+    M = ids.numel()
+    pkv = PackedKV(eng, segments, M, max_keys, llm._body.config.num_hidden_layers, zero_tail_rows=t)
+    out = llm._body(input_ids=ids.view(1, M), position_ids=pos.view(1, M), attention_mask=None, past_key_values=pkv, use_cache=True)
+    if pkv.served != len(pkv.layers):
+        raise RuntimeError(f"glb_short_attention_packed served {pkv.served} of {len(pkv.layers)} layers: an attention module "
+                           "bypassed the attention interface and attended across the packed contexts")
+    enc = PackedEncoding(out, last, M)
+    enc.row_of, enc.live = row_of, live
+    return enc
+
+
 class PrefixLRU:
 
     def __init__(self, budget_bytes, on_remove=None):
diff --git a/genlm-backend_amd/sis.py b/genlm-backend_amd/sis.py
--- a/genlm-backend_amd/sis.py
+++ b/genlm-backend_amd/sis.py
@@ -8,7 +8,8 @@
 from .cache import KVPrefix
 from .engine import check_truncation
 from .fuse import SplitConv1D, split_gemm_all_rows
-from .kv import PACKED_MAX_KEYS, PrefixTable, PromptGroups, SlabKV, SlabRunner, encode_packed, encode_ragged, packed_supported
+from .kv import (PACKED_MAX_KEYS, PrefixTable, PromptGroups, SlabKV, SlabRunner, encode_packed, encode_packed_slots, encode_ragged,
+                 packed_supported)
 from ._lib import MASK_BITS, MASK_NONE
 from .masks import ParticleMasks
 
@@ -131,12 +132,80 @@
         return self.host_s * 1e6 + sum(a.elapsed_time(b) for a, b in self.events) * 1e3
 
 
+HEAD_MAX_AGE = 2
+SLOT_DENSE = (15, 16)
+
+
+def choose_head(step, heads, max_age=HEAD_MAX_AGE, throttle=True):
+    young = [k for k, (at, _, _) in enumerate(heads) if 0 <= step - at <= max_age]
+    landed = [k for k in young if heads[k][1] is None or heads[k][1].query()]
+    if landed:
+        return landed[-1], False
+    if throttle and young:
+        return young[0], True
+    return None
+
+
+def slot_verdict(words, n, rows_needed=0, dense=SLOT_DENSE):
+    U, n_active, _, err = (int(w) for w in words)
+    if err:
+        return "error"
+    if n_active != n:
+        return "finished"
+    if U * dense[1] < dense[0] * n:
+        return "sparse"
+    if U < rows_needed:
+        return "few_rows"
+    return None
+
+
+class HeadLag:
+
+    def __init__(self, device):
+        self.device, self.heads = device, []
+        self._pin, self._row, self._events = None, 0, []
+
+    def clear(self):
+        self._events.extend(e for _, e, _ in self.heads if e is not None)
+        self.heads = []
+
+    def push_known(self, step, words):
+        self.heads.append((step, None, tuple(int(w) for w in words)))
+        self._trim()
+
+    def push(self, step, head_d):
+        if self._pin is None or self._row == self._pin.shape[0]:
+            self._pin, self._row = torch.empty((256, 4), dtype=torch.int32, pin_memory=True), 0
+        row = self._pin[self._row]
+        self._row += 1
+        row.copy_(head_d, non_blocking=True)
+        ev = self._events.pop() if self._events else torch.cuda.Event()
+        ev.record(torch.cuda.current_stream(self.device))
+        self.heads.append((step, ev, row))
+        self._trim()
+        return row
+
+    def _trim(self):
+        while len(self.heads) > HEAD_MAX_AGE + 2:
+            _, e, _ = self.heads.pop(0)
+            if e is not None and e.query():
+                self._events.append(e)
+
+    def wait_last(self):
+        if not self.heads:
+            return None
+        _, e, words = self.heads[-1]
+        if e is not None:
+            e.synchronize()
+        return tuple(int(w) for w in words)
+
+
 class DeviceSIS:
 
     def __init__(self, llm, n_particles, prompt_ids, max_tokens, eos_id, seed=0, rng="philox", rank=0, world=1,
                  dist=None, use_prefix_kv=False, use_particle_kv=False, resample_ess=None, force_collectives=False,
                  share_kv=True, kv_rows=None, kv_in_place=0.75, kv_graph=True, particle_masks=None, migrate_kv=True,
-                 constraint=None, share_prompt_rows=True, proposal_temperature=None, proposal=None):
+                 constraint=None, share_prompt_rows=True, proposal_temperature=None, proposal=None, sync_free=False):
         if constraint is not None and particle_masks is not None:
             raise ValueError("give particle_masks (the caller's bit rows) or constraint (masks made on the device), not both")
         self._propose = proposal_temperature is not None or proposal is not None
@@ -231,6 +300,9 @@
         self.resample_ess = resample_ess
         self.n_resamples = 0
         self.sync_every = 1
+        self.sync_free = bool(sync_free) and self.dev.type == "cuda" and self._groups is not None and self.proposal is None
+        self._lag = HeadLag(self.dev) if self.sync_free else None
+        self.slot_steps, self.dense_fallbacks, self.fallback_reasons = 0, 0, {}
         self.reset()
 
     pkv = property(lambda self: self._kv.pkv)
@@ -264,16 +336,20 @@
         self.last_stats = None
         self.kernel_events = []
         self.outer_events = []
-        self._event_pool = []
+        self._event_pool = getattr(self, "_event_pool", [])
         self._head_cache = None
         self._noise_buf = getattr(self, "_noise_buf", None)
         self._fwd_tokens = None
         self._noise_groups = None
         self._kv_stale = None
         self._row_of_d = torch.full((self.N,), -1, dtype=torch.int32, device=self.dev)
-        self._global_active = torch.tensor(self.N * self.world, dtype=torch.int32, device=self.dev)
+        self._global_active = torch.full((), self.N * self.world, dtype=torch.int32, device=self.dev)
         self.all_weights = None
         self._all_stamp = None
+        self._slot_rows = False
+        if self._lag is not None:
+            self._lag.clear()
+            self._lag.push_known(0, (len(self._groups.lens), self.N, self.N * self.world, 0))
         self._rehash()
 
     def _rehash(self):
@@ -362,7 +438,7 @@
             kw["noise"] = self._parity_noise(self._noise_groups if self._noise_groups is not None else group_of, V)
         if time_kernel:
             if len(self._event_pool) < 2:
-                self._event_pool = eng.timing_events(64)
+                self._event_pool = eng.timing_events(256 if self._lag is not None else 64)
             inner, (e0, e1) = self._event_pool.pop(), self._event_pool.pop()
             e0.record()
             kw["timing_events"] = inner
@@ -393,7 +469,7 @@
         q, self._q_logits = self._q_logits, None
         if time_kernel:
             if len(self._event_pool) < 2:
-                self._event_pool = eng.timing_events(64)
+                self._event_pool = eng.timing_events(256 if self._lag is not None else 64)
             e0, e1 = self._event_pool.pop()
             e0.record()
         dlogw, tok, _ = eng.importance_step(logits, q, proposal_scale=self._q_scale, vocab=logits.shape[-1], row_of=group_of,
@@ -428,6 +504,11 @@
             own = torch.arange(self.N, dtype=torch.int32, device=self.dev)
             return torch.where(done > 0, torch.full_like(own, self.N), own), False
         ids = done if self.constraint is None else self.constraint.mask_rows(self.states, done=done)
+        if self._slot_rows:
+            if self._mask_by_row:
+                own = torch.arange(self.N, dtype=torch.int32, device=self.dev)
+                ids = torch.where(group_of == own, ids, torch.zeros_like(ids))
+            return ids, self._mask_by_row
         if self._mask_by_row and group_of is not None:
             ids = ids[self._rep[:logits.shape[0]].long()].contiguous()
         return ids, self._mask_by_row
@@ -482,11 +563,28 @@
         hashes_eff = torch.where(self.active > 0, self.hashes, self._hash_stub)
         group_of, rep, ng = eng.group_contexts(ctx_flat, self.starts, lengths_eff, hashes=hashes_eff)
         self._rep = rep
-        head = torch.stack([ng[0], self.active.sum().to(torch.int32), self._global_active, eng.error_word()[0]]).cpu()
-        U, n_active, n_global = int(head[0]), int(head[1]), int(head[2])
-        eng.raise_if_failed(int(head[3]))
+        head_d = torch.stack([ng[0], self.active.sum().to(torch.int32), self._global_active, eng.error_word()[0]])
+        l_max = self.max_len_now
+        self._slot_rows = False
+        mode, words = self._lagged_mode(l_max) if self._lag is not None else (None, None)
+        if mode is not None:
+            U_now = self._lag.push(self.t, head_d)[0]
+            if mode == "slot":
+                with split_gemm_all_rows(eng):
+                    enc = encode_packed_slots(llm, (ctx_flat, self.starts, lengths_eff), self.active, group_of, rep, ng, self._grp,
+                                              self._groups, self.t, max_keys=l_max)
+                self._fwd_tokens, self._slot_rows = enc.n_rows, True
+                self.slot_steps += 1
+                self._noise_groups = group_of
+                return self._finish_step(llm._lm_head(enc.last_rows()), enc.row_of, U_now, self.N, words[2], time_kernel, l_max)
+            U, n_active, n_global = words[0], words[1], words[2]
+        else:
+            head = head_d.cpu()
+            U, n_active, n_global = int(head[0]), int(head[1]), int(head[2])
+            eng.raise_if_failed(int(head[3]))
+            if self._lag is not None:
+                self._lag.push_known(self.t, head.tolist())
         base, prefixes = None, None
-        l_max = self.max_len_now
         if self.prefixes is not None and self.t > 0:
             P = self.prefixes
             pref, base = eng.match_prefixes(ctx_flat, self.starts, lengths_eff, P.tokens, P.starts, P.lengths)
@@ -510,12 +608,46 @@
     def _packed_ready(self, U, n_active, l_max):
         if self._groups is None or self.t < 1 or n_active != self.N or l_max > PACKED_MAX_KEYS or self.prefixes is not None:
             return False
+        need = self._split_rows()
+        return need is not None and U * l_max >= need
+
+    def _split_rows(self):
         body = self.llm._body
         ent = self.__dict__.get("_packed_body")
         if ent is None or ent[0] is not body:
             rows = [m.min_rows for m in body.modules() if isinstance(m, SplitConv1D)]
             ent = self._packed_body = (body, max(rows) if rows and packed_supported(self.llm) else None)
-        return ent[1] is not None and U * l_max >= ent[1]
+        return ent[1]
+
+    def _all_split(self):
+        ent = self._packed_body
+        if len(ent) == 2:
+            ent = self._packed_body = ent + (not any(type(m).__name__ == "Conv1D" for m in ent[0].modules()),)
+        return ent[2]
+
+    def _lagged_mode(self, l_max):
+        if self.prefixes is not None or self.collective or self.particle_kv:
+            return None, None
+        heads = self._lag.heads
+        if self.t == 0:
+            known = [w for at, e, w in heads if at == 0 and e is None]
+            return ("known", known[-1]) if known else (None, None)
+        need = self._split_rows()
+        if self.t >= self.max_tokens or l_max > PACKED_MAX_KEYS or need is None or not self._all_split():
+            return None, None
+        pick = choose_head(self.t, heads)
+        why = "no_head"
+        if pick is not None:
+            at, ev, words = heads[pick[0]]
+            if pick[1]:
+                ev.synchronize()
+            words = tuple(int(w) for w in words)
+            why = "first_draw" if at == 0 else slot_verdict(words, self.N, -(-need // l_max))
+            if why is None:
+                return "slot", words
+        self.dense_fallbacks += 1
+        self.fallback_reasons[why] = self.fallback_reasons.get(why, 0) + 1
+        return None, None
 
     def _parity_noise(self, group_of, V):
         N = self.N
@@ -636,6 +768,8 @@
                 self._kv_stale = stale if bool(stale.any().item()) else None
         self._rehash()
         self._recompute_states()
+        if self._lag is not None:
+            self._lag.clear()
         self.n_resamples += 1
         self._exchange()
 
@@ -666,7 +800,13 @@
             steps += 1
             if n_global == 0:
                 break
+        self._settle()
         return steps
+
+    def _settle(self):
+        last = self._lag.wait_last() if self._lag is not None else None
+        if last is not None:
+            self.eng.raise_if_failed(last[3])
 
     @torch.no_grad()
     def rescore(self, llm=None, prompt_ids=None, constraint=None):
@@ -694,6 +834,7 @@
         return llm.batch_sequence_logprobs_device(tokens, lengths, plen, constraint=constraint, forced_at=forced_at)
 
     def results(self):
+        self._settle()
         self.eng.check()
         if self.constraint is not None:
             self.constraint.check()
@@ -765,7 +906,7 @@
 
     def __init__(self, eng, dev, rank, world, dist, n_particles=1024, max_tokens=10, prefix_kv=False, particle_kv=False,
                  model="gpt2", n_prompts=1, resample=False, force_collectives=False, kv_in_place=0.75,
-                 per_particle_masks=False, rng="philox", gemms="library", share_prompt_rows=True):
+                 per_particle_masks=False, rng="philox", gemms="library", share_prompt_rows=True, sync_free=True):
         from .llm import AsyncAmdLM
 
         if model == "gpt2":
@@ -821,7 +962,7 @@
                              seed=1234, rng=rng, rank=rank, world=world, dist=dist, use_prefix_kv=prefix_kv,
                              use_particle_kv=particle_kv, resample_ess=1.0 if resample else None,
                              force_collectives=force_collectives, kv_in_place=kv_in_place, particle_masks=pm,
-                             share_prompt_rows=share_prompt_rows)
+                             share_prompt_rows=share_prompt_rows, sync_free=sync_free)
         self.prefix_kv = prefix_kv
         self.particle_kv = particle_kv
         self.resample = resample
@@ -829,6 +970,7 @@
         self._events = []
         self._outer = []
         self._bytes = []
+        self._lazy_u = []
         self.unique_hist = []
         self.fed_hist = []
         self.flops_hist = []
@@ -847,13 +989,26 @@
             self.sis.reset()
         U, _ = self.sis.step(time_kernel=timed)
         if timed:
-            n_masks = self.N + 1 if self.per_particle_masks else 2
-            self._bytes.append(U * self.V * self.elem + n_masks * ((self.V + 31) // 32) * 4 + self.N * 8
-                               + (self.N * self.V * 4 if self.rng != "philox" else 0))
+            if torch.is_tensor(U):
+                self._lazy_u.append((len(self._bytes), U))
+                U = 0
+            self._bytes.append(self._step_bytes(U))
             self.unique_hist.append(U)
             self.fed_hist.append(int(self.sis.last_stats["l_max"]))
             ls = self.sis.last_stats
             self.flops_hist.append(2.0 * self._lin_w * ls["fwd_tokens"] + 2.0 * self._head_w * ls["head_rows"])
+
+    def _step_bytes(self, U):
+        n_masks = self.N + 1 if self.per_particle_masks else 2
+        return (U * self.V * self.elem + n_masks * ((self.V + 31) // 32) * 4 + self.N * 8
+                + (self.N * self.V * 4 if self.rng != "philox" else 0))
+
+    def _resolve(self):
+        for k, u in self._lazy_u:
+            if k < len(self._bytes):
+                self.unique_hist[k] = int(u)
+                self._bytes[k] = self._step_bytes(int(u))
+        self._lazy_u = []
 
     def _collect(self):
         self._events.extend(self.sis.kernel_events)
@@ -863,12 +1018,15 @@
 
     def kernel_times_us(self):
         self._collect()
+        self._resolve()
         self.kernel_bytes = float(np.mean(self._bytes)) if self._bytes else 0.0
         self.kernel_bytes_each = np.array(self._bytes, dtype=np.float64)
         return np.array([a.elapsed_time(b) * 1e3 for a, b in self._events])
 
     def keep_kernel_times(self, n):
         self._collect()
+        torch.cuda.synchronize(self.sis.dev)
+        self._resolve()
         for name in ("_events", "_outer", "_bytes", "unique_hist", "fed_hist", "flops_hist"):
             setattr(self, name, getattr(self, name)[:n])
 
@@ -876,6 +1034,9 @@
         return np.array([a.elapsed_time(b) * 1e3 for a, b in self._outer])
 
     def config(self):
+        if self._lazy_u:
+            torch.cuda.synchronize(self.sis.dev)
+            self._resolve()
         return {"workload": f"SIS step: {self.N} particles/GPU, {self.model_name}, prompt len 8, <=10 new "
                             "tokens, " + (f"{self.N} per-particle bit masks (standing still: handed over raw at the first step, prepared from the second on)" if self.per_particle_masks
                                           else "2 shared bit masks") + ", device-resident population, "
diff --git a/include/glb.h b/include/glb.h
--- a/include/glb.h
+++ b/include/glb.h
@@ -196,6 +196,12 @@
                                int64_t max_keys, int64_t head_dim, float scale, int32_t dtype, void *out, uint32_t *err_word,
                                void *hip_stream);
 
+int glb_short_attention_packed_slots(const void *q, int64_t q_stride_row, int64_t q_stride_head, const void *k,
+                                     int64_t k_stride_row, int64_t k_stride_head, const void *v, int64_t v_stride_row,
+                                     int64_t v_stride_head, const int32_t *plan, int64_t n_segments, int64_t n_rows,
+                                     int64_t heads, int64_t kv_heads, int64_t max_keys, int64_t head_dim, float scale,
+                                     int32_t dtype, int64_t zero_tail_rows, void *out, uint32_t *err_word, void *hip_stream);
+
 size_t glb_resample_workspace(int64_t n);
 int glb_resample_systematic(const float *log_weights, int64_t n, uint64_t seed, uint64_t offset,
                             int32_t *out_ancestors, float *out_stats, void *workspace, size_t workspace_bytes,
@@ -347,6 +353,31 @@
   int32_t *ends;
 } glb_packed_plan_args;
 int glb_packed_plan(const glb_packed_plan_args *args, void *hip_stream);
+
+typedef struct glb_packed_plan_slots_args {
+  uint32_t struct_size;
+  int64_t n_tokens, n_contexts, n_groups, n_pre, slot_rows, pos_cap;
+  const int32_t *tokens;
+  const int64_t *starts;
+  const int32_t *lengths;
+  const int32_t *active;
+  const int32_t *group_of;
+  const int32_t *rep;
+  const int32_t *n_groups_found;
+  const int32_t *grp;
+  const int32_t *group_starts;
+  const int32_t *group_lens;
+  const int32_t *group_segments;
+  const int64_t *group_ids;
+  const int64_t *group_pos;
+  int32_t *segments;
+  int64_t *ids;
+  int64_t *pos;
+  int64_t *last;
+  int32_t *row_of;
+  int32_t *live_count;
+} glb_packed_plan_slots_args;
+int glb_packed_plan_slots(const glb_packed_plan_slots_args *args, void *hip_stream);
 
 typedef struct glb_lora_job {
   uint32_t struct_size;
```

After: 148,100, median of 6. No clear change (+1.2%).
